# wgurecky/CORRLA_RS

Measured on AMD Instinct MI355X. Metric: RSVD GFLOP/s on 16k x 16k f32 rank-128, higher is better.
Workload: dtype f32

## Files before the change

### corrla_rs_amd/_lib.py

```python
import ctypes as C
import os

PKG = os.path.dirname(os.path.abspath(__file__))
LIB_PATH = os.environ.get("CORRLA_RSVD_LIB") or os.path.join(PKG, "lib", "libcorrla_rsvd.so")

i64, u64, u32, i32, dbl, flt = C.c_int64, C.c_uint64, C.c_uint32, C.c_int32, C.c_double, C.c_float
vp = C.c_void_p

OK, EINVAL, ENOMEM, EHIP, ECOMM, ENUMERIC, ENODEV = range(7)
OMEGA_ON_DEVICE = 0x1
PCA_CENTER_FUSED = 0x2
PCA_CENTER_COPY = 0x4
QR_HOUSEHOLDER = 0x8
SEED_EXPLICIT = 0x10
POWER_FUSED = 0x20
SHARD_COLS = 0x40
SKETCH_BF16X3 = 0x80
SKETCH_BF16X6 = 0x100
PCA_STANDARDIZE = 0x200
COV_CORRELATION = 0x1
COV_NO_CENTER = 0x2
COV_ROUTE_INPLACE, COV_ROUTE_INPLACE_CHECKED, COV_ROUTE_REPACKED = 1, 2, 3
COV_ROUTES = {COV_ROUTE_INPLACE: "inplace", COV_ROUTE_INPLACE_CHECKED: "inplace_checked", COV_ROUTE_REPACKED: "repacked"}
PCA_APPLY_OWN_MEANS = 0x400
# ... 27 lines not shown
                ("scales_out", vp)]


class Timings(C.Structure):
    _fields_ = [("total_ms", dbl), ("sketch_ms", dbl), ("power_ms", dbl), ("qr_ms", dbl), ("project_ms", dbl),
                ("small_svd_ms", dbl), ("finalize_ms", dbl), ("qr_passes", i32), ("n_collectives", i32),
                ("sketch_kernel_ms", dbl), ("host_enqueue_ms", dbl), ("collective_bytes", dbl), ("n_mixed_products", i32),
                ("n_bf16_products", i32), ("knn_ms", dbl), ("fit_ms", dbl)]


def _sigs():
    s = {
        "corrla_version": (C.c_char_p, []),
        "corrla_last_error": (C.c_char_p, []),
        "corrla_device_count": (C.c_int, []),
        "corrla_ctx_create": (C.c_int, [C.c_int, C.POINTER(vp)]),
        "corrla_ctx_destroy": (None, [vp]),
        "corrla_ctx_synchronize": (C.c_int, [vp]),
        "corrla_ctx_get_timings": (C.c_int, [vp, C.POINTER(Timings)]),
        "corrla_ctx_set_phase_timings": (C.c_int, [vp, C.c_int]),
        "corrla_ctx_comm_info": (C.c_int, [vp, C.POINTER(C.c_int), C.POINTER(C.c_int)]),
        "corrla_comm_unique_id": (C.c_int, [vp]),
        "corrla_ctx_comm_init": (C.c_int, [vp, vp, C.c_int, C.c_int]),
        "corrla_ctx_last_pca_apply": (C.c_int, [vp, C.POINTER(C.c_int), C.POINTER(C.c_int)]),
        "corrla_ctx_last_polyfit": (C.c_int, [vp, C.POINTER(C.c_int)]),
        "corrla_ctx_last_kde": (C.c_int, [vp, C.POINTER(C.c_int)]),
        "corrla_ctx_last_dirichlet": (C.c_int, [vp, C.POINTER(C.c_int)]),
        "corrla_ctx_last_mvn": (C.c_int, [vp, C.POINTER(C.c_int)]),
    }
    s["corrla_dirichlet_draws_f64"] = s["corrla_dirichlet_draws_dev_f64"] = (C.c_int, [vp, vp, i64, dbl, u64, i64, i64, vp, i64])
    s["corrla_dirichlet_sample_f64"] = s["corrla_dirichlet_sample_dev_f64"] = (
        C.c_int, [vp, vp, vp, i64, dbl, u64, i64, i64, i64, vp, i64, C.POINTER(i64), C.POINTER(i64)])
    s["corrla_lu_solve_f64"] = (C.c_int, [vp, vp, i64, i64, vp, i64, i64, vp, i64])
    s["corrla_lu_solve_dev_f64"] = (C.c_int, [vp, vp, i64, i64, vp, i64, i64, vp])
    s["corrla_rbffit_system_f64"] = s["corrla_rbffit_system_dev_f64"] = (C.c_int, [vp, vp, i64, i64, i64, C.c_int, dbl, C.c_int, vp, i64])
    s["corrla_rbffit_f64"] = s["corrla_rbffit_dev_f64"] = (C.c_int, [vp, vp, i64, i64, i64, vp, i64, i64, C.c_int, dbl, C.c_int, vp, i64])
    s["corrla_ctx_last_solve"] = (C.c_int, [vp, C.POINTER(C.c_int), C.POINTER(i64), C.POINTER(dbl), C.POINTER(dbl)])
    s["corrla_chol_factor_f64"] = (C.c_int, [vp, vp, i64, i64, vp, i64])
    s["corrla_chol_factor_dev_f64"] = (C.c_int, [vp, vp, i64, i64])
    s["corrla_chol_solve_f64"] = (C.c_int, [vp, vp, i64, i64, vp, i64, i64, vp, i64])
    s["corrla_chol_solve_dev_f64"] = (C.c_int, [vp, vp, i64, i64, vp, i64, i64])
    s["corrla_ctx_last_chol"] = (C.c_int, [vp, C.POINTER(C.c_int), C.POINTER(i64), C.POINTER(dbl), C.POINTER(dbl), C.POINTER(dbl)])
    for suf, sc in (("f32", flt), ("f64", dbl)):
        rsvd = [vp, vp, i64, i64, i64, i64, i64, i64, i64, C.POINTER(Opts), vp, i64, vp, vp, i64]
        s["corrla_rsvd_" + suf] = (C.c_int, rsvd)
        s["corrla_rsvd_dev_" + suf] = (C.c_int, rsvd)
        s["corrla_rsvd_sharded_dev_" + suf] = (C.c_int, rsvd)
        pca = [vp, vp, i64, i64, i64, i64, i64, i64, i64, C.POINTER(Opts), vp, vp, vp, i64]
        s["corrla_pca_" + suf] = (C.c_int, pca)
        s["corrla_pca_dev_" + suf] = (C.c_int, pca)
        s["corrla_pca_sharded_dev_" + suf] = (C.c_int, pca)
        pw = [vp, vp, i64, i64, i64, i64, i64, i64, C.POINTER(Opts), vp, i64]
        s["corrla_power_iter_" + suf] = (C.c_int, pw)
        s["corrla_power_iter_dev_" + suf] = (C.c_int, pw)
        s["corrla_matmul_dev_" + suf] = (C.c_int, [vp, C.c_int, vp, i64, i64, i64, i64, vp, i64, i64, sc, vp, i64])
        rsvd_csr = [vp, vp, vp, vp, i64, i64, i64, i64, i64, i64, C.POINTER(Opts), vp, i64, vp, vp, i64]
        s["corrla_rsvd_csr_" + suf] = (C.c_int, rsvd_csr)
        s["corrla_rsvd_csr_dev_" + suf] = (C.c_int, rsvd_csr)
        pca_csr = [vp, vp, vp, vp, i64, i64, i64, i64, i64, i64, C.POINTER(Opts), vp, vp, vp, i64]
        s["corrla_pca_csr_" + suf] = (C.c_int, pca_csr)
        s["corrla_pca_csr_dev_" + suf] = (C.c_int, pca_csr)
        s["corrla_spmm_csr_dev_" + suf] = (C.c_int, [vp, C.c_int, vp, vp, vp, i64, i64, i64, vp, i64, i64, sc, vp, i64])
        cov = [vp, vp, i64, i64, i64, i64, u64, C.c_int, vp, vp, vp, i64, C.POINTER(C.c_int)]
        s["corrla_cov_" + suf] = (C.c_int, cov)
        s["corrla_cov_dev_" + suf] = (C.c_int, cov)
        model = [vp, vp, vp, i64, i64, u64, vp, i64, vp, vp]
        s["corrla_pca_transform_" + suf] = s["corrla_pca_transform_dev_" + suf] = (C.c_int, [vp, vp, i64, i64, i64, i64] + model)
        s["corrla_pca_transform_csr_" + suf] = s["corrla_pca_transform_csr_dev_" + suf] = (C.c_int, [vp, vp, vp, vp, i64, i64, i64] + model)
        inverse = [vp, vp, i64, i64, i64, vp, vp, vp, i64, i64, vp, i64]
        s["corrla_pca_inverse_" + suf] = s["corrla_pca_inverse_dev_" + suf] = (C.c_int, inverse)
        points = [vp, vp, i64, i64, vp, i64, i64, i64, C.c_int, dbl]
        s["corrla_rbf_matrix_" + suf] = s["corrla_rbf_matrix_dev_" + suf] = (C.c_int, points + [vp, i64])
        s["corrla_rbf_apply_" + suf] = s["corrla_rbf_apply_dev_" + suf] = (C.c_int, points + [C.c_int, vp, i64, i64, vp, i64])
        gram = [vp, vp, i64, i64, i64, vp, i64, i64, C.c_int, C.c_int, vp, i64, vp, vp]
        s["corrla_polyfit_gram_" + suf] = s["corrla_polyfit_gram_dev_" + suf] = (C.c_int, gram)
        peval = [vp, vp, i64, i64, i64, vp, i64, i64, C.c_int, vp, i64, vp, i64]
        s["corrla_poly_eval_" + suf] = s["corrla_poly_eval_dev_" + suf] = (C.c_int, peval)
        kde = [vp, vp, i64, i64, vp, i64, i64]
        s["corrla_kde_eval_" + suf] = s["corrla_kde_eval_dev_" + suf] = (C.c_int, kde + [dbl, C.c_int, vp, i64])
        s["corrla_kde_nll_" + suf] = s["corrla_kde_nll_dev_" + suf] = (C.c_int, kde + [vp, i64, vp, vp])
        s["corrla_mvn_sample_" + suf] = s["corrla_mvn_sample_dev_" + suf] = (C.c_int, [vp, i64, i64, i64, vp, i64, vp, u64, i64, C.c_int, vp, i64])
        s["corrla_sandwich_diag_" + suf] = s["corrla_sandwich_diag_dev_" + suf] = (C.c_int, [vp, vp, i64, i64, i64, vp, i64, vp])
        s["corrla_fill_normal_dev_" + suf] =(C.c_int, [vp, vp, i64, i64, i64, i64, u64, i64, i64])
        s["corrla_time_sketch_dev_" + suf] = (C.c_int, [vp, vp, i64, i64, i64, i64, vp, i64, i64, vp, i64, C.c_int,
                                                         C.POINTER(dbl)])
    s["corrla_rsvd_bf16"] = s["corrla_rsvd_dev_bf16"] = s["corrla_rsvd_f32"]
    s["corrla_pca_bf16"] = s["corrla_pca_dev_bf16"] = s["corrla_pca_f32"]
    s["corrla_matmul_dev_bf16"] = s["corrla_matmul_dev_f32"]
    grad = [vp, vp, i64, i64, vp, vp, i64, C.c_int, i64, dbl, vp, i64, C.POINTER(C.c_int)]
    s["corrla_grad_mat_f64"] = (C.c_int, grad)
    s["corrla_grad_mat_dev_f64"] = (C.c_int, grad)
    return s


SIGNATURES = _sigs()
_lib = None


class CorrlaError(RuntimeError):
    def __init__(self, code, msg):
        super().__init__(f"corrla_rsvd error {code}: {msg}")
        self.code = code


def load():
    global _lib
    if _lib is not None:
        return _lib
    if not os.path.exists(LIB_PATH):
        raise ImportError(
            f"{LIB_PATH} is missing: build it with `python -m corrla_rs_amd.build` (hipcc, gfx950). "
            "corrla_rs_amd has no CPU fallback.")
    try:
        import torch
    except ImportError:
        pass
    lib = C.CDLL(LIB_PATH, mode=C.RTLD_GLOBAL)
    for name, (res, args) in SIGNATURES.items():
        fn = getattr(lib, name)
        fn.restype = res
        fn.argtypes = args
    _lib = lib
    return lib


def check(code):
    if code != OK:
        msg = load().corrla_last_error().decode("utf-8", "replace")
        if code == EINVAL:
            raise ValueError(f"corrla_rsvd: {msg}")
        if code == ENOMEM:
            raise MemoryError(f"corrla_rsvd: {msg}")
        raise CorrlaError(code, msg)
```

### corrla_rs_amd/api.py

```python
import atexit
import ctypes as C
import sys
import threading
import weakref

import numpy as np

from . import _lib as L

__all__ = ["Context", "default_context", "rsvd", "random_svd", "power_iter", "rpca", "PcaRsvd", "algorithmic_flops"]


def _is_torch(x):
    return type(x).__module__.split(".")[0] == "torch"


def _is_torch_csr(x):
    return _is_torch(x) and str(getattr(x, "layout", "")) == "torch.sparse_csr"


def _is_sparse(x):
    if isinstance(x, tuple):
        def nd(v):
            return v.ndim if hasattr(v, "ndim") else np.ndim(v)
# ... 1000 lines not shown
        L.check(self._entry(name, True, in_dtype or xt.dtype)(self._h, 1 if trans else 0, *_c_args(operand), xc.data_ptr(), xin, l, float(beta),
                                                  res.data_ptr(), xout))
        return res.t()

    def spmm(self, a_csr, x, trans=False, beta=1.0):
        import torch
        vals, ci, rp, (m, n), on_dev = _as_csr(a_csr)
        dev = torch.device(f"cuda:{self.device}")
        if not on_dev:
            vals, ci, rp = (torch.from_numpy(v).to(dev) for v in (vals, ci, rp))
        xt = x if _is_torch(x) else torch.as_tensor(np.asarray(x))
        xt = xt.to(device=dev, dtype=vals.dtype)
        if xt.dim() != 2 or xt.shape[0] != (m if trans else n):
            raise ValueError(f"x must have {m if trans else n} rows")
        return self._run_product("corrla_spmm_csr_", (vals, ci, rp, m, n, int(vals.shape[0])),
                                 m, n, xt, trans, beta)

    def matmul(self, a, x, trans=False, beta=1.0):
        m, n = a.shape
        if _is_bf16(x):
            raise ValueError("matmul: x must be float32 or float64 (only the matrix a may be bfloat16)")
        if _is_bf16(a):
            if not str(x.dtype).endswith("float32"):
                raise ValueError("matmul: a bfloat16 a takes a float32 x")
            assert x.shape[0] == (m if trans else n)
            return self._run_product("corrla_matmul_", (a, m, n, *a.stride()), m, n, x, trans, beta, in_dtype=a.dtype)
        assert x.shape[0] == (m if trans else n) and x.dtype == a.dtype
        return self._run_product("corrla_matmul_", (a, m, n, *a.stride()), m, n, x, trans, beta)

    def grad_mat(self, x_mat, y, est_order, n_nbrs, x_query=None, *, scale=1.0):
        est_order, n_nbrs = int(est_order), int(n_nbrs)
        nreg = C.c_int(0)
        if _is_torch(x_mat) and x_mat.is_cuda:
            import torch
            x = x_mat.to(torch.float64).contiguous()
            yv = (y if _is_torch(y) else torch.as_tensor(np.asarray(y))).to(device=x.device, dtype=torch.float64).reshape(-1).contiguous()
            xq = x if x_query is None else x_query.to(device=x.device, dtype=torch.float64).contiguous()
            if x.dim() != 2 or xq.dim() != 2 or xq.shape[1] != x.shape[1] or yv.numel() != x.shape[0]:
                raise ValueError("x_mat (n, k), y (n,), x_query (n_q, k) expected")
            g = torch.empty((xq.shape[0], x.shape[1]), dtype=torch.float64, device=x.device)
            _sync_stream(x)
            L.check(self._lib.corrla_grad_mat_dev_f64(self._h, x.data_ptr(), x.shape[0], x.shape[1], yv.data_ptr(), xq.data_ptr(),
                                                      xq.shape[0], est_order, n_nbrs, float(scale), g.data_ptr(), x.shape[1],
                                                      C.byref(nreg)))
            return g.t(), nreg.value
        x = np.ascontiguousarray(np.asarray(x_mat, dtype=np.float64))
        yv = np.ascontiguousarray(np.asarray(y, dtype=np.float64).reshape(-1))
        xq = x if x_query is None else np.ascontiguousarray(np.asarray(x_query, dtype=np.float64))
        if x.ndim != 2 or xq.ndim != 2 or xq.shape[1] != x.shape[1] or yv.size != x.shape[0]:
            raise ValueError("x_mat (n, k), y (n,), x_query (n_q, k) expected")
        g = np.empty((xq.shape[0], x.shape[1]), dtype=np.float64)
        L.check(self._lib.corrla_grad_mat_f64(self._h, x.ctypes.data, x.shape[0], x.shape[1], yv.ctypes.data, xq.ctypes.data,
                                              xq.shape[0], est_order, n_nbrs, float(scale), g.ctypes.data, x.shape[1],
                                              C.byref(nreg)))
        return g.T, nreg.value

    def power_iter(self, a_mat, omega_rank, n_iter, *, seed=None, omega=None, qr=None):
        _reject_bf16(a_mat, "power_iter")
        a = np.asarray(a_mat)
        if a.ndim != 2:
            raise ValueError("a_mat must be 2-D")
        if a.dtype != np.float32:
            a = a.astype(np.float64, copy=False)
        m, n = a.shape
        w = int(omega_rank)
        rs, cs = _strides(a)
        o, keep = self._opts(seed, omega, n, w, a.dtype, False, self._qr_flag(qr))
        q = _empty_colmajor(a, m, max(w, 1))
        fn = self._entry("corrla_power_iter_", False, a.dtype)
        L.check(fn(self._h, a.ctypes.data, m, n, rs, cs, w, int(n_iter), C.byref(o) if o is not None else None,
                   q.ctypes.data, m))
        del keep
        return q

    def fill_normal(self, t, seed, row0=0, global_cols=None):
        rows, cols = t.shape
        rs, cs = t.stride()
        _sync_stream(t)
        fn = self._entry("corrla_fill_normal_", True, t.dtype)
        L.check(fn(self._h, t.data_ptr(), rows, cols, rs, cs, int(seed), int(row0),
                   int(global_cols if global_cols is not None else cols)))
        return t

    def time_sketch(self, a, x, reps=10):
        import torch
        m, n = a.shape
        rs, cs = a.stride()
        l = x.shape[1]
        xc = x.t().contiguous()
        y = torch.empty((l, m), dtype=a.dtype, device=a.device)
        ms = C.c_double()
        _sync_stream(a)
        fn = self._entry("corrla_time_sketch_", True, a.dtype)
        L.check(fn(self._h, a.data_ptr(), m, n, rs, cs, xc.data_ptr(), n, l, y.data_ptr(), m, int(reps), C.byref(ms)))
        return ms.value, y.t()


_default = None
_default_lock = threading.Lock()


def default_context():
    global _default
    with _default_lock:
        if _default is None:
            _default = Context(0)
        return _default


def rsvd(a_mat, n_rank, n_iters, n_oversamples, *, seed=None, omega=None, ctx=None, qr=None):
    return (ctx or default_context()).rsvd(a_mat, n_rank, n_iters, n_oversamples, seed=seed, omega=omega, qr=qr)


def random_svd(a_mat, omega_rank, n_iter, n_oversamples, *, seed=None, omega=None, ctx=None, qr=None):
    return rsvd(a_mat, omega_rank, n_iter, n_oversamples, seed=seed, omega=omega, ctx=ctx, qr=qr)


def power_iter(a_mat, omega_rank, n_iter, *, seed=None, omega=None, ctx=None, qr=None):
    return (ctx or default_context()).power_iter(a_mat, omega_rank, n_iter, seed=seed, omega=omega, qr=qr)


def rpca(a_mat, n_rank, n_iters=None, n_oversamples=None, *, seed=None, omega=None, ctx=None, standardize=False):
    del n_iters, n_oversamples
    if not _check_standardize(standardize):
        _means, s, comps = (ctx or default_context()).pca(a_mat, n_rank, seed=seed, omega=omega)
    else:
        _means, s, comps, _scales = (ctx or default_context()).pca(a_mat, n_rank, seed=seed, omega=omega, standardize=True)
    return s, comps


def normal_stream_host(seed, first, n, r, dtype=np.float64):
    dtype = np.dtype(dtype)
    if dtype not in (np.float32, np.float64):
        raise ValueError(f"dtype must be float32 or float64, got {dtype}")
    n, r, seed, first = int(n), int(r), int(seed), int(first)
    if n < 0 or r < 1 or first < 0 or (first + n) * r >= 1 << 63:
        raise ValueError("need n >= 0, r >= 1, first >= 0 and (first + n) * r < 2^63")
    m32, sh = np.uint64(0xFFFFFFFF), np.uint64(32)
    t = (np.uint64(first) + np.arange(n, dtype=np.uint64))[:, None] * np.uint64(r) + np.arange(r, dtype=np.uint64)[None, :]
    c0, c1, c2, c3 = t & m32, t >> sh, np.zeros_like(t), np.zeros_like(t)
    k0, k1 = np.uint64(seed & 0xFFFFFFFF), np.uint64((seed >> 32) & 0xFFFFFFFF)
    for _ in range(10):
        p0, p1 = np.uint64(0xD2511F53) * c0, np.uint64(0xCD9E8D57) * c2
        c0, c1, c2, c3 = (p1 >> sh) ^ c1 ^ k0, p1 & m32, (p0 >> sh) ^ c3 ^ k1, p0 & m32
        k0, k1 = (k0 + np.uint64(0x9E3779B9)) & m32, (k1 + np.uint64(0xBB67AE85)) & m32
    if dtype == np.float64:
        u1 = ((((c0 << sh) | c1) >> np.uint64(11)).astype(np.float64) + 0.5) * 2.0 ** -53
        u2 = ((((c2 << sh) | c3) >> np.uint64(11)).astype(np.float64) + 0.5) * 2.0 ** -53
    else:
        u1 = ((c0 >> np.uint64(8)).astype(np.float32) + np.float32(0.5)) * np.float32(2.0 ** -24)
        u2 = ((c1 >> np.uint64(8)).astype(np.float32) + np.float32(0.5)) * np.float32(2.0 ** -24)
    x = dtype.type(2.0) * u2
    y = np.where(x > 1.0, dtype.type(2.0) - x, x)
    pi = dtype.type(np.pi)
    c = np.where(y < 0.25, np.cos(pi * y), np.where(y > 0.75, -np.cos(pi * (dtype.type(1.0) - y)), np.sin(pi * (dtype.type(0.5) - y))))
    return (np.sqrt(dtype.type(-2.0) * np.log(u1)) * c).astype(dtype)


class PcaRsvd:

    def __init__(self, x_mat, rank, *, seed=None, omega=None, ctx=None, standardize=False):
        self.pca_rank = int(rank)
        x = x_mat if _is_sparse(x_mat) or (_is_torch(x_mat) and x_mat.is_cuda) else np.asarray(x_mat)
        self._ctx = ctx
        self.n_samples = int(x[3][0] if isinstance(x, tuple) else x.shape[0])
        self.scales_ = None
# ... 83 lines not shown
```

### corrla_rs_amd/csrc/capi_impl.hpp

```cpp
#pragma once
#include <cstddef>
#include <cstdint>
#include <cstring>
#include <string>
#include <vector>

#include "../../include/corrla_rsvd.h"
#include "call_spans.hpp"
#include "driver.hpp"
#include "rbf_plan.hpp"
#include "polyfit_plan.hpp"
#include "kde_plan.hpp"
#include "dirichlet_plan.hpp"
#include "mvn_plan.hpp"
#include "chol_plan.hpp"
#include "lu_plan.hpp"

namespace corrla {

inline std::string& last_error_slot() {
  static thread_local std::string msg;
  return msg;
}

// ... 140 lines not shown
    dev.begin_call();
    begun = true;
    stage();
  };
  if (!sharded) {
    prepare();
    return;
  }
  if (dev.nranks() < 1) throw Error(ST_ECOMM, "communicator not initialised");
  int local = ST_OK;
  std::string local_msg;
  try {
    prepare();
  } catch (const Error& e) {
    local = e.code;
    local_msg = e.what();
  } catch (const std::bad_alloc&) {
    local = ST_ENOMEM;
    local_msg = "host allocation failed";
  }
  if (!begun) dev.begin_call();
  const int agreed = dev.sharded_handshake(local);
  if (local != ST_OK) throw Error(local, local_msg);
  if (agreed != ST_OK)
    throw Error(agreed, "sharded call abandoned: another rank failed before the first collective (status " + std::to_string(agreed) +
                            "); this rank's arguments were valid");
}

template <class Dev, class T>
inline void finish_call(RsvdDriver<Dev, T>& drv, Dev& dev, Timings* tm_out, bool with_sketch_kernel_ms) {
  PhaseTimer fin;
  drv.phase(drv.tm.finalize_ms, fin);
  dev.phase_end();
  dev.end_call();
  dev.phase_resolve(&drv.tm.total_ms);
  drv.tm.n_collectives = dev.n_collectives;
  drv.tm.collective_bytes = dev.collective_bytes;
  if (with_sketch_kernel_ms) drv.tm.sketch_kernel_ms = dev.event_elapsed_ms(0, 1);
  if (tm_out) *tm_out = drv.tm;
}

template <class T>
struct RsvdCall {
  bool host_ptrs;
  int64_t m, rank, n_iter, n_oversamples;
  const corrla_opts* opts;
  T* u;
  int64_t ldu;
  T* s;
  T* vt;
  int64_t ldvt;
  Timings* tm_out;
  bool profile;
  bool sharded = false, sparse = false, fat = false, empty_shard = false;
  bool bf16 = false;
};

template <class Dev, class T, class Validate, class Stage>
inline void rsvd_body(Dev& dev, const RsvdCall<T>& c, Validate&& validate, Stage&& stage) {
  const bool shard_cols = c.sharded && c.fat;
  const int64_t k = c.rank;
  RunOpts ro;
  TallA<T> ta;
  bool u_in_place = false;
  int64_t l = 0;
  Skinny<T> ut, vtall;
  T* s_dev = nullptr;
  prepare_call(
      dev, c.sharded,
      [&] {
        if ((!c.u && !(c.empty_shard && !shard_cols)) || !c.s || (!c.vt && !(c.empty_shard && shard_cols)))
          throw Error(ST_EINVAL, "output pointer is NULL");
        validate();
        if (c.ldu < c.m) throw Error(ST_EINVAL, "ldu < m");
        if (c.ldvt < c.rank) throw Error(ST_EINVAL, "ldvt < rank");
        ro = call_opts(c.opts, c.host_ptrs, c.sharded, c.sparse || c.bf16);
        draw_seed(dev, ro);
      },
      [&] {
        ta = stage();
        l = std::min<int64_t>(c.rank + c.n_oversamples, ta.nt);
        if (ro.omega && ro.omega_ld < ta.nt) throw Error(ST_EINVAL, "omega_ld < min(m, n)");
        u_in_place = !c.fat && !c.host_ptrs && !c.empty_shard;
        ut = u_in_place ? caller_skinny(c.u, ta.mt, k, c.ldu) : dev.template alloc_skinny<T>(ta.mt, k);
        vtall = dev.template alloc_skinny<T>(ta.nt, k);
        s_dev = dev.template alloc_scalar<T>((int)k);
      });
  RsvdDriver<Dev, T> drv(dev, c.profile);
  if (c.empty_shard) drv.m_local_override_ = 0;
  drv.random_svd_tall(ta, k, l, c.n_iter, ro, ut, s_dev, vtall, [&] {
    if (!c.fat) {
      if (!u_in_place && !c.empty_shard) dev.copy_out(ut, k, c.u, c.ldu, false, c.host_ptrs);
      dev.copy_out(vtall, k, c.vt, c.ldvt, true, c.host_ptrs);
    } else {
      dev.copy_out(vtall, k, c.u, c.ldu, false, c.host_ptrs);
      if (!c.empty_shard) dev.copy_out(ut, k, c.vt, c.ldvt, true, c.host_ptrs);
    }
    dev.copy_values_out(s_dev, k, c.s, c.host_ptrs);
  });
  finish_call(drv, dev, c.tm_out, true);
}

template <class Dev, class T>
inline void rsvd_entry(Dev& dev, bool host_ptrs, bool sharded, const T* a, int64_t m, int64_t n, int64_t rs, int64_t cs,
                       int64_t rank, int64_t n_iter, int64_t n_oversamples, const corrla_opts* opts, T* u, int64_t ldu,
                       T* s, T* vt, int64_t ldvt, Timings* tm_out, bool profile) {
  const bool shard_cols = sharded && opts && (opts->flags & CORRLA_SHARD_COLS) != 0;
  const bool empty_shard = sharded && m >= 0 && n >= 0 && (shard_cols ? (n == 0 && m >= 1) : (m == 0 && n >= 1));
  const int64_t short_side = shard_cols ? m : n;
  RsvdCall<T> c{host_ptrs, m, rank, n_iter, n_oversamples, opts, u, ldu, s, vt, ldvt, tm_out, profile};
  c.sharded = sharded;
  c.fat = sharded ? shard_cols : m < n;
  c.empty_shard = empty_shard;
  rsvd_body(
      dev, c,
      [&] {
        if (!empty_shard) validate_matrix(a, m, n, rs, cs);
        if (!sharded && opts && (opts->flags & CORRLA_SHARD_COLS)) throw Error(ST_EINVAL, "CORRLA_SHARD_COLS is only valid for sharded entry points");
        if (sharded) {
          if (rank < 1 || rank > short_side) throw Error(ST_EINVAL, "rank must be in [1, short side] for the sharded path");
          if (n_iter < 0 || n_oversamples < 0) throw Error(ST_EINVAL, "n_iter and n_oversamples must be >= 0");
        } else {
          validate_rank(m, n, rank, n_iter, n_oversamples);
        }
      },
      [&] {
        if (empty_shard) return zero_row_tall<Dev, T>(dev, short_side);
        return shard_cols ? stage_input<Dev, T>(dev, host_ptrs, a, n, m, cs, rs, true)
                          : stage_input<Dev, T>(dev, host_ptrs, a, m, n, rs, cs, sharded);
      });
}

inline void need_two_samples(int64_t m) {
  if (m < 2) throw Error(ST_EINVAL, "PCA needs at least two samples");
}

template <class T>
struct PcaCall {
  bool host_ptrs;
  int64_t m, n, rank, n_iter, n_oversamples;
  const corrla_opts* opts;
  T* means;
  T* s;
  T* comps;
  int64_t ldc;
  Timings* tm_out;
  bool profile;
  bool sharded = false, sparse = false;
  bool bf16 = false;
};

template <class Dev, class T, class Validate, class Stage>
inline void pca_body(Dev& dev, const PcaCall<T>& c, Validate&& validate, Stage&& stage) {
  RunOpts ro;
  TallA<T> ta;
  T* scales_out = nullptr;
  prepare_call(
      dev, c.sharded,
      [&] {
        if (!c.means || !c.s || !c.comps) throw Error(ST_EINVAL, "output pointer is NULL");
        validate();
        if (c.ldc < c.rank) throw Error(ST_EINVAL, "ldc < rank");
        if (c.sparse) need_two_samples(c.m);
        ro = call_opts(c.opts, c.host_ptrs, c.sharded, c.sparse || c.bf16, true);
        if (ro.pca_standardize && !dev_has_colvar<Dev>::value)
          throw Error(ST_EINVAL, "CORRLA_PCA_STANDARDIZE: this backend has no column-variance kernels");
        if (ro.pca_standardize && c.opts->struct_size >= sizeof(corrla_opts)) scales_out = (T*)c.opts->scales_out;
        if (c.sparse && ro.pca_center == 2)
          throw Error(ST_EINVAL, "CORRLA_PCA_CENTER_COPY on CSR input: a centred copy would densify the matrix (use the fused centring)");
        draw_seed(dev, ro);
      },
      [&] { ta = stage(); });
  const int64_t m_global = c.sharded ? dev.allreduce_sum_host(c.m) : c.m;
  need_two_samples(m_global);
  const bool fat = !c.sharded && c.m < c.n;
  RsvdDriver<Dev, T> drv(dev, c.profile);
  Skinny<T> mu = drv.column_means(ta, fat, m_global, c.sharded);
  const bool data_cols_along_mem_cols = (ta.row_major != fat);
  Skinny<T> sd, inv_sd;
  if (ro.pca_standardize) {
    if constexpr (dev_has_colvar<Dev>::value) {
// ... 939 lines not shown
```

### corrla_rs_amd/csrc/core_svd_stage.hpp

```cpp
#pragma once
#include "core_svd_plan.hpp"
#include "hip_backend.hpp"

namespace corrla {

template <class T>
struct CoreSvdCall {
  const Skinny<T>& c;
  int64_t l, k;
  Skinny<T>&m1, &m2;
  T* s_dev;
  void* conv_status;
};

namespace core_svd_stage {

template <class T>
using RingEs = std::integer_sequence<int, 8, 12, 16, sizeof(T) == 4 ? 20 : 18>;
constexpr int kMaxNc = 9;

template <class T>
inline void set_lds_limits() {
  for_each_of(RingEs<T>{}, [](auto e) { lds_limit((const void*)k::jacobi_ring_w_kernel<T, decltype(e)::value, 8>, k::kLdsMaxBytes); });
  lds_limit((const void*)k::jacobi_block_round_kernel<T>, k::kLdsMaxBytes);
// ... 78 lines not shown
  int* bad = a.conv_status ? nullptr : dev.alloc_flags(1);
  hipLaunchKernelGGL((k::core_finite_check_kernel<T>), dim3(1), dim3(1024), 0, dev.stream, (const T*)a.c.p, a.c.ld, (int)a.l,
                     (k::CholStatus*)a.conv_status, bad, sexp_out);
  CORRLA_HIP(hipGetLastError());
  if (bad) {
    int h = 0;
    dev.read_flags(bad, 1, &h);
    if (h) throw Error(ST_ENUMERIC, "non-finite core matrix in small SVD");
  }
}

template <class T>
inline void block(HipDev& dev, const CoreSvdCall<T>& a, const CoreSvdPlan& plan, const int* sexp) {
  const CoreSvdPlan::Block& p = plan.blk;
  const int64_t ld = p.rows_pad;
  T* wj = (T*)dev.alloc_bytes(p.ws_bytes);
  T* vj = (T*)dev.alloc_bytes(p.ws_bytes);
  k::JacobiCtl* ctl = (k::JacobiCtl*)dev.alloc_bytes(sizeof(k::JacobiCtl));
  hipLaunchKernelGGL((k::jacobi_init_kernel<T>), dim3(64), dim3(256), 0, dev.stream, (const T*)a.c.p, a.c.ld, (int)a.l, wj, ld, vj,
                     ld, p.cols_pad, p.rows_pad, ctl, sexp);
  for (int sw = 0; sw < p.max_sweeps; ++sw) {
    for (int round = 0; round < p.nb - 1; ++round)
      hipLaunchKernelGGL((k::jacobi_block_round_kernel<T>), dim3(p.nb / 2), dim3(256), p.round_lds, dev.stream, wj, ld, vj, ld,
                         p.rows_pad, p.nb, round, p.inner, ctl);
    hipLaunchKernelGGL(k::jacobi_sweep_end_kernel, dim3(1), dim3(1), 0, dev.stream, ctl, (float)plan.tol_early);
  }
  hipLaunchKernelGGL((k::jacobi_finish_kernel<T>), dim3(1), dim3(1024), p.fin_lds, dev.stream, (const T*)wj, ld, (const T*)vj,
                     ld, (int)a.l, a.m1.p, a.m1.ld, a.m2.p, a.m2.ld, a.s_dev, (int)a.k, sexp);
  CORRLA_HIP(hipGetLastError());
  if (env_int("CORRLA_DEBUG", 0)) {
    k::JacobiCtl h;
    CORRLA_HIP(hipMemcpyAsync(&h, ctl, sizeof(h), hipMemcpyDeviceToHost, dev.stream));
    dev.sync();
    std::fprintf(stderr, "[corrla] block jacobi l=%d nb=%d sweeps=%u done=%u\n", (int)a.l, p.nb, h.sweeps, h.done);
  }
}

template <class T>
inline void ring(HipDev& dev, const CoreSvdCall<T>& a, const CoreSvdPlan& plan) {
  static_assert(sizeof(k::RotEntry<T>) == 2 * sizeof(T), "CoreSvdPlan::Ring::rot_bytes");
  const CoreSvdPlan::Ring& p = plan.ring;
  int* info = (int*)dev.alloc_bytes(sizeof(int) * 4);
  k::RotEntry<T>* rot = (k::RotEntry<T>*)dev.alloc_bytes(p.rot_bytes);
  int* rank_g = (int*)dev.alloc_bytes(p.rank_bytes);
  const T tol = (T)plan.tol, tol_early = (T)plan.tol_early;
  with_one_of(RingEs<T>{}, plan.ring_e, [&](auto e) {
    hipLaunchKernelGGL((k::jacobi_ring_w_kernel<T, decltype(e)::value, 8>), dim3(1), dim3(p.block), p.lds, dev.stream, (const T*)a.c.p,
                       a.c.ld, (int)a.l, a.m2.p, a.m2.ld, a.s_dev, (int)a.k, tol, tol_early, p.max_sw, rot, rank_g, info);
  });
  CORRLA_HIP(hipGetLastError());
  hipLaunchKernelGGL((k::jacobi_replay_v_kernel<T>), dim3(p.replay_grid), dim3(256), 0, dev.stream, (const k::RotEntry<T>*)rot,
                     (const int*)info, (const int*)rank_g, (int)a.l, (int)a.k, a.m1.p, a.m1.ld);
  CORRLA_HIP(hipGetLastError());
  if (env_int("CORRLA_DEBUG", 0)) {
    int h[4] = {0, 0, 0, 0};
    CORRLA_HIP(hipMemcpyAsync(h, info, sizeof(int), hipMemcpyDeviceToHost, dev.stream));
    dev.sync();
    std::fprintf(stderr, "[corrla] jacobi_svd (ring) l=%d sweeps=%d\n", (int)a.l, h[0]);
  }
}

inline CoreSvdKnobs knobs_from_env() {
  CoreSvdKnobs kn;
  kn.mode = std::getenv("CORRLA_SVD");
  kn.host_svd = env_int("CORRLA_HOST_SVD", 0) != 0;
  kn.jmc_min_l = env_int("CORRLA_JMC_MIN_L", kn.jmc_min_l);
  kn.jmc_max_b = std::min(32, std::max(2, env_int("CORRLA_JMC_MAX_B", kn.jmc_max_b)));
  kn.jmc_local = env_int("CORRLA_JMC_LOCAL", kn.jmc_local);
  kn.jmc_np = env_int("CORRLA_JMC_NP", kn.jmc_np);
  kn.jmc_sweeps_f32 = env_int("CORRLA_JMC_SWEEPS", kn.jmc_sweeps_f32);
  kn.jmc_sweeps_f64 = env_int("CORRLA_JMC_SWEEPS", kn.jmc_sweeps_f64);
  kn.jmc_force_v = env_int("CORRLA_JMC_FORCE_V", 0) != 0;
  kn.strict = env_int("CORRLA_JACOBI_STRICT", 0) != 0;
  kn.block_sweeps = env_int("CORRLA_JACOBI_SWEEPS", kn.block_sweeps);
  kn.ring_sweeps = env_int("CORRLA_JACOBI_SWEEPS", kn.ring_sweeps);
  kn.block_inner = env_int("CORRLA_JACOBI_INNER", kn.block_inner);
  return kn;
}

}

template <class T>
void HipDev::small_svd(const Skinny<T>& c, int64_t l, int64_t k, Skinny<T>& m1, Skinny<T>& m2, T* s_dev, void* conv_status) {
  if (conv_status) memset_zero(conv_status, sizeof(k::CholStatus));
  const CoreSvdCall<T> a{c, l, k, m1, m2, s_dev, conv_status};
  const CoreSvdPlan plan = core_svd_plan((int)sizeof(T), l, k, core_svd_stage::knobs_from_env(), svd_state_, conv_status != nullptr);
  switch (plan.family) {
    case CoreSvd::kMultiWg:
      core_svd_stage::multi_wg(*this, a, plan);
      return;
    case CoreSvd::kHost:
      small_svd_host(*this, c, l, k, m1, m2, s_dev);
      return;
    case CoreSvd::kBlock: {
      int* sexp = (int*)alloc_bytes(sizeof(int));
      core_svd_stage::finite_check(*this, a, sexp);
      core_svd_stage::block(*this, a, plan, sexp);
      return;
    }
    case CoreSvd::kRing:
      core_svd_stage::finite_check(*this, a);
      core_svd_stage::ring(*this, a, plan);
      return;
  }
}

}
```

### corrla_rs_amd/csrc/corrla_rsvd.hip

```cpp
#include <mutex>

#include "capi_impl.hpp"
#include "colstat_stage.hpp"
#include "core_svd_stage.hpp"
#include "cov_stage.hpp"
#include "dirichlet_stage.hpp"
#include "grad_stage.hpp"
#include "hip_backend.hpp"
#include "kde_stage.hpp"
#include "chol_stage.hpp"
#include "lu_stage.hpp"
#include "mvn_stage.hpp"
#include "pca_apply_stage.hpp"
#include "polyfit_stage.hpp"
#include "rbf_stage.hpp"
#include "tall_stage.hpp"
#include "thinq_stage.hpp"

using namespace corrla;

struct corrla_ctx {
  HipDev dev;
  Timings last;
  std::mutex mu;
  bool profile;
  pca_apply_stage::Ran pca_apply;
  polyfit_stage::Ran polyfit;
  kde_stage::Ran kde;
  dirichlet_stage::Ran dirichlet;
  mvn_stage::Ran mvn;
  lu_stage::Ran lu;
  chol_stage::Ran chol;
  explicit corrla_ctx(int ordinal) : dev(ordinal), profile(env_int("CORRLA_PROFILE_PHASES", 0) != 0) {}
};

namespace {
inline corrla_ctx* need(corrla_ctx* c) {
  if (!c) throw Error(ST_EINVAL, "ctx is NULL");
  return c;
}
template <class F>
inline void locked_call(corrla_ctx* c, F&& f) {
  std::lock_guard<std::mutex> lk(c->mu);
  try {
    f();
  } catch (...) {
    (void)hipSetDevice(c->dev.device);
    if (c->dev.stream) (void)hipStreamSynchronize(c->dev.stream);
    (void)hipGetLastError();
    throw;
  }
}

template <class F, class After>
inline corrla_status ctx_call(corrla_ctx* ctx, F&& f, After&& after) {
  return guarded([&] {
    corrla_ctx* c = need(ctx);
    locked_call(c, [&] { f(*c); });
    after(*c);
  });
}
template <class F>
inline corrla_status ctx_call(corrla_ctx* ctx, F&& f) {
  return ctx_call(ctx, f, [](corrla_ctx&) {});
}
inline void debug_qr_breakdown(const corrla_ctx& c) {
  if (c.profile && env_int("CORRLA_DEBUG", 0))
    std::fprintf(stderr, "[corrla] qr breakdown (ms): gram %.3f  download+check %.3f  host chol/inv %.3f  upload+apply %.3f  (%d passes)\n",
                 c.last.qr_gram_ms, c.last.qr_down_ms, c.last.qr_host_ms, c.last.qr_apply_ms, c.last.qr_passes);
}
template <class T>
corrla_status fill_c(corrla_ctx* ctx, T* p, int64_t rows, int64_t cols, int64_t rs, int64_t cs, uint64_t seed,
                     int64_t row0, int64_t global_cols) {
  return guarded([&] {
    corrla_ctx* c = need(ctx);
    if (!p) throw Error(ST_EINVAL, "p is NULL");
    if (rows < 0 || cols < 0 || rs < 0 || cs < 0 || global_cols < cols) throw Error(ST_EINVAL, "bad fill_normal shape");
    std::lock_guard<std::mutex> lk(c->mu);
    CORRLA_HIP(hipSetDevice(c->dev.device));
    c->dev.fill_normal(p, rows, cols, rs, cs, seed, row0, global_cols);
    c->dev.sync();
  });
}
template <class T>
corrla_status time_sketch_c(corrla_ctx* ctx, const T* a, int64_t m, int64_t n, int64_t rs, int64_t cs, const T* x,
                            int64_t ldx, int64_t l, T* y, int64_t ldy, int reps, double* avg_ms) {
  return guarded([&] {
    corrla_ctx* c = need(ctx);
    if (!x || !y || !avg_ms) throw Error(ST_EINVAL, "NULL argument");
    if (reps < 1 || l < 1 || ldx < n || ldy < m) throw Error(ST_EINVAL, "bad time_sketch arguments");
    std::lock_guard<std::mutex> lk(c->mu);
    HipDev& dev = c->dev;
    dev.begin_call();
    TallA<T> ta = stage_input<HipDev, T>(dev, false, a, m, n, rs, cs, true);
    RsvdDriver<HipDev, T> drv(dev, false);
    drv.mixed_planes_ = parse_opts(nullptr, true).mixed_planes;
    Skinny<T> xs = dev.alloc_skinny<T>(n, l);
    dev.copy_in_skinny(x, ldx, xs);
    Skinny<T> out = dev.alloc_skinny<T>(m, l);
    *avg_ms = dev.time_on_stream(reps, [&] { drv.a_times(ta, xs, out, nullptr); });
    dev.copy_out(out, l, y, ldy, false, false);
    dev.end_call();
  });
}
}

extern "C" {

CORRLA_API const char* corrla_version(void) { return "corrla_rsvd 0.1.0 gfx950"; }
CORRLA_API const char* corrla_last_error(void) { return last_error_slot().c_str(); }
CORRLA_API int corrla_device_count(void) {
  int n = 0;
  if (hipGetDeviceCount(&n) != hipSuccess) {
    (void)hipGetLastError();
    return 0;
  }
  return n;
}

CORRLA_API corrla_status corrla_ctx_create(int device_ordinal, corrla_ctx** out) {
  return guarded([&] {
    if (!out) throw Error(ST_EINVAL, "out is NULL");
    *out = nullptr;
    *out = new corrla_ctx(device_ordinal);
  });
}
CORRLA_API void corrla_ctx_destroy(corrla_ctx* ctx) { delete ctx; }
CORRLA_API corrla_status corrla_ctx_synchronize(corrla_ctx* ctx) {
  return guarded([&] { need(ctx)->dev.sync(); });
}
CORRLA_API corrla_status corrla_ctx_comm_info(corrla_ctx* ctx, int* rank, int* nranks) {
  return guarded([&] {
    corrla_ctx* c = need(ctx);
    if (!rank || !nranks) throw Error(ST_EINVAL, "NULL argument");
    std::lock_guard<std::mutex> lk(c->mu);
    c->dev.comm_info(rank, nranks);
  });
}
CORRLA_API corrla_status corrla_ctx_set_phase_timings(corrla_ctx* ctx, int on) {
  return guarded([&] {
    corrla_ctx* c = need(ctx);
    std::lock_guard<std::mutex> lk(c->mu);
    c->dev.set_phase_events(on != 0);
  });
}
CORRLA_API corrla_status corrla_ctx_get_timings(corrla_ctx* ctx, corrla_timings* out) {
  return guarded([&] {
    corrla_ctx* c = need(ctx);
    if (!out) throw Error(ST_EINVAL, "out is NULL");
    const Timings& t = c->last;
    out->total_ms = t.total_ms;
    out->sketch_ms = t.sketch_ms;
    out->power_ms = t.power_ms;
    out->qr_ms = t.qr_ms;
    out->project_ms = t.project_ms;
    out->small_svd_ms = t.small_svd_ms;
    out->finalize_ms = t.finalize_ms;
    out->qr_passes = t.qr_passes;
    out->n_collectives = t.n_collectives;
    out->collective_bytes = t.collective_bytes;
    out->sketch_kernel_ms = t.sketch_kernel_ms;
    out->host_enqueue_ms = t.host_enqueue_ms;
    out->n_mixed_products = t.n_mixed_products;
    out->n_bf16_products = t.n_bf16_products;
    out->knn_ms = t.knn_ms;
    out->fit_ms = t.fit_ms;
  });
}

#define CORRLA_DENSE(T, A) const T *A, int64_t m, int64_t n, int64_t rs, int64_t cs
#define CORRLA_CSR_A(T) const T *values, const int32_t *col_idx, const int64_t *row_ptr, int64_t m, int64_t n, int64_t nnz
#define CORRLA_RSVD_REST(T) int64_t rank, int64_t n_iter, int64_t p, const corrla_opts *o, T *u, int64_t ldu, T *s, T *vt, int64_t ldvt
#define CORRLA_PCA_REST(T) int64_t rank, int64_t n_iter, int64_t p, const corrla_opts *o, T *means, T *s, T *comps, int64_t ldc
#define CORRLA_PRODUCT_REST(T) const T *x, int64_t ldx, int64_t l, T beta, T *res, int64_t ldres

#define CORRLA_DEFINE_RSVD(NAME, T, HOST, SHARDED)                                                                      \
  CORRLA_API corrla_status NAME(corrla_ctx* ctx, CORRLA_DENSE(T, a), CORRLA_RSVD_REST(T)) {                              \
    return ctx_call(ctx, [&](corrla_ctx& c) {                                                                           \
      rsvd_entry<HipDev, T>(c.dev, HOST, SHARDED, a, m, n, rs, cs, rank, n_iter, p, o, u, ldu, s, vt, ldvt, &c.last,     \
                            c.profile);                                                                                 \
    }, debug_qr_breakdown);                                                                                             \
  }
#define CORRLA_DEFINE_PCA(NAME, T, HOST, SHARDED)                                                                       \
  CORRLA_API corrla_status NAME(corrla_ctx* ctx, CORRLA_DENSE(T, x), CORRLA_PCA_REST(T)) {                             \
    return ctx_call(ctx, [&](corrla_ctx& c) {                                                                           \
      pca_entry<HipDev, T>(c.dev, HOST, x, m, n, rs, cs, rank, n_iter, p, o, means, s, comps, ldc, &c.last, c.profile,   \
                           SHARDED);                                                                                    \
    });                                                                                                                 \
  }
#define CORRLA_DEFINE_POWER(NAME, T, HOST)                                                                              \
  CORRLA_API corrla_status NAME(corrla_ctx* ctx, CORRLA_DENSE(T, a), int64_t width, int64_t n_iter, const corrla_opts* o, \
                                T* q, int64_t ldq) {                                                                    \
    return ctx_call(ctx, [&](corrla_ctx& c) {                                                                           \
      power_iter_entry<HipDev, T>(c.dev, HOST, a, m, n, rs, cs, width, n_iter, o, q, ldq);                              \
    });                                                                                                                 \
  }

#define CORRLA_DEFINE(SUF, T)                                                                                          \
  CORRLA_DEFINE_RSVD(corrla_rsvd_##SUF, T, true, false)                                                                \
  CORRLA_DEFINE_RSVD(corrla_rsvd_dev_##SUF, T, false, false)                                                           \
  CORRLA_DEFINE_RSVD(corrla_rsvd_sharded_dev_##SUF, T, false, true)                                                    \
  CORRLA_DEFINE_PCA(corrla_pca_##SUF, T, true, false)                                                                  \
  CORRLA_DEFINE_PCA(corrla_pca_dev_##SUF, T, false, false)                                                             \
  CORRLA_DEFINE_PCA(corrla_pca_sharded_dev_##SUF, T, false, true)                                                      \
  CORRLA_DEFINE_POWER(corrla_power_iter_##SUF, T, true)                                                                \
  CORRLA_DEFINE_POWER(corrla_power_iter_dev_##SUF, T, false)                                                           \
  CORRLA_API corrla_status corrla_matmul_dev_##SUF(corrla_ctx* ctx, int trans, CORRLA_DENSE(T, a), CORRLA_PRODUCT_REST(T)) { \
    return ctx_call(ctx, [&](corrla_ctx& c) {                                                                          \
      matmul_entry<HipDev, T>(c.dev, trans, a, m, n, rs, cs, x, ldx, l, beta, res, ldres, &c.last);                    \
    });                                                                                                                \
  }                                                                                                                    \
  CORRLA_API corrla_status corrla_fill_normal_dev_##SUF(corrla_ctx* ctx, T* p, int64_t rows, int64_t cols, int64_t rs,            \
                                             int64_t cs, uint64_t seed, int64_t row0, int64_t global_cols) {           \
    return fill_c<T>(ctx, p, rows, cols, rs, cs, seed, row0, global_cols);                                             \
  }                                                                                                                    \
  CORRLA_API corrla_status corrla_time_sketch_dev_##SUF(corrla_ctx* ctx, const T* a, int64_t m, int64_t n, int64_t rs,            \
                                             int64_t cs, const T* x, int64_t ldx, int64_t l, T* y, int64_t ldy,        \
                                             int reps, double* avg_ms) {                                               \
    return time_sketch_c<T>(ctx, a, m, n, rs, cs, x, ldx, l, y, ldy, reps, avg_ms);                                    \
  }

CORRLA_DEFINE(f32, float)
CORRLA_DEFINE(f64, double)

#define CORRLA_DEFINE_RSVD_CSR(NAME, T, HOST)                                                                           \
  CORRLA_API corrla_status NAME(corrla_ctx* ctx, CORRLA_CSR_A(T), CORRLA_RSVD_REST(T)) {                                \
    return ctx_call(ctx, [&](corrla_ctx& c) {                                                                           \
      rsvd_csr_entry<HipDev, T>(c.dev, HOST, values, col_idx, row_ptr, m, n, nnz, rank, n_iter, p, o, u, ldu, s, vt,     \
                                ldvt, &c.last, c.profile);                                                              \
    });                                                                                                                 \
  }
#define CORRLA_DEFINE_PCA_CSR(NAME, T, HOST)                                                                            \
  CORRLA_API corrla_status NAME(corrla_ctx* ctx, CORRLA_CSR_A(T), CORRLA_PCA_REST(T)) {                                 \
    return ctx_call(ctx, [&](corrla_ctx& c) {                                                                           \
      pca_csr_entry<HipDev, T>(c.dev, HOST, values, col_idx, row_ptr, m, n, nnz, rank, n_iter, p, o, means, s, comps,    \
                               ldc, &c.last, c.profile);                                                                \
    });                                                                                                                 \
  }

#define CORRLA_DEFINE_CSR(SUF, T)                                                                                      \
  CORRLA_DEFINE_RSVD_CSR(corrla_rsvd_csr_##SUF, T, true)                                                               \
  CORRLA_DEFINE_RSVD_CSR(corrla_rsvd_csr_dev_##SUF, T, false)                                                          \
  CORRLA_DEFINE_PCA_CSR(corrla_pca_csr_##SUF, T, true)                                                                 \
  CORRLA_DEFINE_PCA_CSR(corrla_pca_csr_dev_##SUF, T, false)                                                            \
  CORRLA_API corrla_status corrla_spmm_csr_dev_##SUF(corrla_ctx* ctx, int trans, CORRLA_CSR_A(T), CORRLA_PRODUCT_REST(T)) { \
    return ctx_call(ctx, [&](corrla_ctx& c) {                                                                          \
      spmm_entry<HipDev, T>(c.dev, trans, values, col_idx, row_ptr, m, n, nnz, x, ldx, l, beta, res, ldres);           \
    });                                                                                                                \
  }

CORRLA_DEFINE_CSR(f32, float)
CORRLA_DEFINE_CSR(f64, double)

#define CORRLA_DEFINE_RSVD_BF16(NAME, HOST)                                                                             \
  CORRLA_API corrla_status NAME(corrla_ctx* ctx, CORRLA_DENSE(uint16_t, a), CORRLA_RSVD_REST(float)) {                  \
    return ctx_call(ctx, [&](corrla_ctx& c) {                                                                           \
      rsvd_bf16_entry<HipDev>(c.dev, HOST, a, m, n, rs, cs, rank, n_iter, p, o, u, ldu, s, vt, ldvt, &c.last, c.profile); \
    });                                                                                                                 \
  }
#define CORRLA_DEFINE_PCA_BF16(NAME, HOST)                                                                              \
  CORRLA_API corrla_status NAME(corrla_ctx* ctx, CORRLA_DENSE(uint16_t, x), CORRLA_PCA_REST(float)) {                   \
    return ctx_call(ctx, [&](corrla_ctx& c) {                                                                           \
      pca_bf16_entry<HipDev>(c.dev, HOST, x, m, n, rs, cs, rank, n_iter, p, o, means, s, comps, ldc, &c.last, c.profile); \
    });                                                                                                                 \
  }
CORRLA_DEFINE_RSVD_BF16(corrla_rsvd_bf16, true)
CORRLA_DEFINE_RSVD_BF16(corrla_rsvd_dev_bf16, false)
CORRLA_DEFINE_PCA_BF16(corrla_pca_bf16, true)
CORRLA_DEFINE_PCA_BF16(corrla_pca_dev_bf16, false)
CORRLA_API corrla_status corrla_matmul_dev_bf16(corrla_ctx* ctx, int trans, CORRLA_DENSE(uint16_t, a), CORRLA_PRODUCT_REST(float)) {
  return ctx_call(ctx, [&](corrla_ctx& c) {
    matmul_bf16_entry<HipDev>(c.dev, trans, a, m, n, rs, cs, x, ldx, l, beta, res, ldres, &c.last);
  });
}

#define CORRLA_DEFINE_COV(NAME, T, HOST)                                                                                \
  CORRLA_API corrla_status NAME(corrla_ctx* ctx, CORRLA_DENSE(T, x), uint64_t flags, int ddof, T* means_out, T* scales_out, \
                                T* c, int64_t ldc, int* route_out) {                                                    \
    return ctx_call(ctx, [&](corrla_ctx& cx) {                                                                          \
      const CovCall<T> call{x, m, n, rs, cs, flags, ddof, means_out, scales_out, c, ldc, route_out};                    \
      cov_entry<HipDev, T>(cx.dev, call, [&] { cov_stage::run<T>(cx.dev, HOST, call); });                               \
    });                                                                                                                 \
  }
CORRLA_DEFINE_COV(corrla_cov_f32, float, true)
CORRLA_DEFINE_COV(corrla_cov_f64, double, true)
CORRLA_DEFINE_COV(corrla_cov_dev_f32, float, false)
CORRLA_DEFINE_COV(corrla_cov_dev_f64, double, false)

#define CORRLA_PCA_MODEL(T) const T *means, const T *scales, const T *components, int64_t ldc, int64_t k, uint64_t flags, T *scores, \
                            int64_t ld_scores, T *resid_out, T *means_out
#define CORRLA_PCA_MODEL_CALL(T) PcaTransformCall<T>{m, n, means, scales, components, ldc, k, flags, scores, ld_scores, resid_out, means_out}
#define CORRLA_DEFINE_PCA_TRANSFORM(NAME, T, HOST)                                                                      \
  CORRLA_API corrla_status NAME(corrla_ctx* ctx, CORRLA_DENSE(T, x), CORRLA_PCA_MODEL(T)) {                             \
    return ctx_call(ctx, [&](corrla_ctx& cx) {                                                                          \
      cx.pca_apply = pca_apply_stage::Ran();                                                                            \
      const PcaTransformCall<T> c = CORRLA_PCA_MODEL_CALL(T);                                                           \
      if (!x) throw Error(ST_EINVAL, "pca_transform: x is NULL");                                                       \
      if (m < 1 || n < 1) throw Error(ST_EINVAL, "pca_transform: m and n must be >= 1");                                \
// ... 323 lines not shown
```

### corrla_rs_amd/csrc/driver.hpp

```cpp
#pragma once
#include <cstdio>
#include <chrono>
#include <cmath>
#include <cstdint>
#include <cstring>
#include <limits>
#include <stdexcept>
#include <string>
#include <functional>
#include <type_traits>
#include <vector>

#include "gemm_plan.hpp"
#include "small_linalg.hpp"
#include "thinq_plan.hpp"

namespace corrla {

struct Error : std::runtime_error {
  int code;
  Error(int c, const std::string& m) : std::runtime_error(m), code(c) {}
};
enum { ST_OK = 0, ST_EINVAL = 1, ST_ENOMEM = 2, ST_EHIP = 3, ST_ECOMM = 4, ST_ENUMERIC = 5, ST_ENODEV = 6 };

// ... 15 lines not shown
template <class T>
struct Big {
  const T* p = nullptr;
  int64_t rows = 0, cols = 0, ld = 0, cols_readable = 0;
};

template <class T>
inline Big<T> as_rowmajor_transposed(const Skinny<T>& y, int64_t ncols) {
  Big<T> b;
  b.p = y.p;
  b.rows = ncols;
  b.cols = y.rows;
  b.ld = y.ld;
  b.cols_readable = y.ld;
  return b;
}

template <class T>
struct CsrView {
  const T* val = nullptr;
  const int32_t* ci = nullptr;
  const int64_t* rp = nullptr;
  int64_t rows = 0, cols = 0, nnz = 0;
  int64_t n_long = 0, n_chunks = 0;
  const int64_t* long_row = nullptr;
  const int64_t* long_base = nullptr;
  const int32_t* chunk_long = nullptr;
};

template <class D, class = void>
struct dev_has_spmm : std::false_type {};
template <class D>
struct dev_has_spmm<D, std::void_t<decltype(D::kHasSpmm)>> : std::true_type {};

template <class D, class = void>
struct dev_has_bf16in : std::false_type {};
template <class D>
struct dev_has_bf16in<D, std::void_t<decltype(D::kHasBf16In)>> : std::true_type {};

template <class D, class = void>
struct dev_has_colvar : std::false_type {};
template <class D>
struct dev_has_colvar<D, std::void_t<decltype(D::kHasColVar)>> : std::true_type {};

template <class D, class = void>
struct dev_has_syrk : std::false_type {};
template <class D>
struct dev_has_syrk<D, std::void_t<decltype(D::kHasSyrk)>> : std::true_type {};

template <class D, class = void>
struct dev_has_pca_apply : std::false_type {};
template <class D>
struct dev_has_pca_apply<D, std::void_t<decltype(D::kHasPcaApply)>> : std::true_type {};

template <class D, class = void>
struct dev_has_rbf : std::false_type {};
template <class D>
struct dev_has_rbf<D, std::void_t<decltype(D::kHasRbf)>> : std::true_type {};

template <class D, class = void>
struct dev_has_polyfit : std::false_type {};
template <class D>
struct dev_has_polyfit<D, std::void_t<decltype(D::kHasPolyfit)>> : std::true_type {};
template <class D, class = void>
struct dev_has_kde : std::false_type {};
template <class D>
struct dev_has_kde<D, std::void_t<decltype(D::kHasKde)>> : std::true_type {};
template <class D, class = void>
struct dev_has_dirichlet : std::false_type {};
template <class D>
struct dev_has_dirichlet<D, std::void_t<decltype(D::kHasDirichlet)>> : std::true_type {};
template <class D, class = void>
struct dev_has_mvn : std::false_type {};
template <class D>
struct dev_has_mvn<D, std::void_t<decltype(D::kHasMvn)>> : std::true_type {};
template <class D, class = void>
struct dev_has_lu : std::false_type {};
template <class D>
struct dev_has_lu<D, std::void_t<decltype(D::kHasLu)>> : std::true_type {};
template <class D, class = void>
struct dev_has_chol : std::false_type {};
template <class D>
struct dev_has_chol<D, std::void_t<decltype(D::kHasChol)>> : std::true_type {};

template <class T>
struct TallA {
  Big<T> mem;
  bool row_major = true;
  int64_t mt = 0, nt = 0;
  const T* mu_short = nullptr;
  const T* mu_tall = nullptr;
  const T* inv_sd_short = nullptr;
  const T* inv_sd_tall = nullptr;
  bool sparse = false;
  CsrView<T> csr, csr_t;
  bool bf16 = false;
  Big<uint16_t> mem16;
};

struct RunOpts {
  uint64_t seed = 0x5eedull;
  bool seed_explicit = false;
  const void* omega = nullptr;
  int64_t omega_ld = 0;
  bool omega_on_device = false;
  bool sharded = false;
  int pca_center = 0;
  bool pca_standardize = false;
  bool qr_householder = false;
  bool power_fused = false;
  int mixed_planes = 0;
  bool mixed_project = true;
  int poison_core = 0;
};
constexpr int kFlagNonFinite = 2, kFlagNullCols = 4;

struct Timings {
  double total_ms = 0, sketch_ms = 0, power_ms = 0, qr_ms = 0, project_ms = 0, small_svd_ms = 0, finalize_ms = 0;
  double host_enqueue_ms = 0;
  int qr_passes = 0;
  int n_collectives = 0;
  double collective_bytes = 0;
  double knn_ms = 0, fit_ms = 0;
  int n_mixed_products = 0;
  int n_bf16_products = 0;
  double qr_gram_ms = 0, qr_down_ms = 0, qr_host_ms = 0, qr_apply_ms = 0;
  double sketch_kernel_ms = 0;
};

struct PhaseTimer {
  using clk = std::chrono::steady_clock;
  clk::time_point t0;
  PhaseTimer() : t0(clk::now()) {}
  double lap() {
    auto t1 = clk::now();
    double ms = std::chrono::duration<double, std::milli>(t1 - t0).count();
    t0 = t1;
    return ms;
  }
};

template <class Dev, class T>
struct RsvdDriver {
  Dev& dev;
  Timings tm;
  bool profile_phases;
  bool qr_householder = false;
  static constexpr const T* kNone = nullptr;

  explicit RsvdDriver(Dev& d, bool profile = false) : dev(d), profile_phases(profile) {}

  int mixed_planes_ = 0;
  void sparse_times(const CsrView<T>& s, const Skinny<T>& x, Skinny<T>& y, const T* scale_dev) {
    if constexpr (dev_has_spmm<Dev>::value)
      dev.spmm(s, x, y, scale_dev);
    else
      throw Error(ST_EINVAL, "this backend has no SpMM kernels: sparse operands are not supported");
  }
  void bf16_times(bool tn, const Big<uint16_t>& r, const Skinny<T>& x, Skinny<T>& y, const T* scale_dev) {
    if constexpr (dev_has_bf16in<Dev>::value && std::is_same<T, float>::value)
      dev.gemm_bf16a(tn, r, x, y, scale_dev), ++tm.n_bf16_products;
    else
      throw Error(ST_EINVAL, "this backend has no bf16-input kernels: bf16 operands are not supported");
  }
  Skinny<T> scale_ws_;
  void set_scale_workspace(const Skinny<T>& ws) { scale_ws_ = ws; }
// ... 96 lines not shown
      p.record = record;
      return p;
    }
  };
  struct Attempt {
    bool defer = false;
    void* st_pool = nullptr;
    int st_slots = 0, st_used = 0;
    int* flags_pool = nullptr;
    int flags_cap = 0, flags_used = 0;
    std::vector<Pending> pending;
    bool dirty = false;
  } att_;
  void* status_record(int i) const { return (char*)att_.st_pool + (size_t)i * kStatusBytes; }
  int64_t m_local_ = 0, m_global_ = -1;
  int64_t m_local_override_ = -1;
  int64_t global_rows(bool sharded) {
    if (!sharded) return m_local_;
    if (m_global_ < 0) m_global_ = dev.allreduce_sum_host(m_local_);
    return m_global_;
  }

  int hh_short_shards_ = -1;
  bool householder_usable(const Skinny<T>& y, bool sharded) {
    if (!qr_householder) return false;
    if (!sharded) return y.rows >= y.cols;
    if (hh_short_shards_ < 0) hh_short_shards_ = (int)dev.allreduce_sum_host(m_local_ < y.cols ? 1 : 0);
    return hh_short_shards_ == 0;
  }
  void householder_panel(Skinny<T>& y, Skinny<T>& tmp, bool sharded) {
    const int64_t l = y.cols;
    auto h = dev.householder_up(y, tmp);
    if (!sharded) {
      dev.householder_down(h, y, tmp);
      return;
    }
    const int64_t np = dev.nranks(), rk = dev.rank();
    Skinny<T> stack = dev.template alloc_skinny<T>(np * l, l), t2 = dev.template alloc_skinny<T>(np * l, l);
    Skinny<T> rv, cv;
    rv.p = h.r_root();
    rv.rows = rv.cols = rv.ld = rv.cols_alloc = l;
    dev.copy_block(rv, 0, 0, l, l, stack, rk * l, 0);
    dev.allreduce(stack.p, (size_t)stack.ld * (size_t)stack.cols_alloc);
    dev.householder_thin_q(stack, t2);
    cv.p = (T*)dev.alloc_zeroed_bytes((size_t)l * (size_t)l * sizeof(T));
    cv.rows = cv.cols = cv.ld = cv.cols_alloc = l;
    dev.copy_block(stack, rk * l, 0, l, l, cv, 0, 0);
    dev.householder_down(h, y, tmp, (const T*)cv.p);
  }
  void householder_thin_q_any_width(Skinny<T>& y, Skinny<T>& tmp, bool sharded) {
    const int64_t l = y.cols, m = y.rows;
    const int64_t w = hh_column_blocks(l, dev.template householder_max_width<T>()).w;
    if (w == l) {
      householder_panel(y, tmp, sharded);
      return;
    }
    std::vector<double> th;
    for (int64_t c0 = 0; c0 < l; c0 += w) {
      const int64_t wb = std::min(w, l - c0);
      Skinny<T> yb = dev.template alloc_skinny<T>(m, wb), tb = dev.template alloc_skinny<T>(m, wb);
      Skinny<T> pb = dev.template alloc_skinny<T>(m, wb);
      dev.copy_block(y, 0, c0, m, wb, yb, 0, 0);
      for (int pass = 0; pass < 5; ++pass) {
        double overlap2 = 0.0;
        if (c0 > 0) {
          Skinny<T> t = dev.template alloc_skinny<T>(c0, wb);
          dev.gemm_nn(as_rowmajor_transposed(y, c0), yb, t, kNone);
          if (sharded) dev.allreduce(t.p, (size_t)t.ld * (size_t)t.cols_alloc);
          if (pass >= 1) {
            th.resize((size_t)(c0 * wb));
            dev.download_skinny(t, c0, wb, th.data());
            for (double v : th) overlap2 += v * v;
          }
          dev.gemm_tn(as_rowmajor_transposed(y, c0), t, pb, kNone);
          dev.sub_inplace(yb, pb);
        }
        householder_panel(yb, tb, sharded);
        if (c0 == 0 || (pass >= 1 && overlap2 <= 0.25)) break;
      }
      dev.copy_block(yb, 0, 0, m, wb, y, 0, c0);
    }
  }

  int64_t orthonormalize(Skinny<T>& y, Skinny<T>& tmp, bool sharded, bool rough = false) {
    const int64_t l = y.cols;
    if (householder_usable(y, sharded)) {
      PhaseTimer qt0;
      householder_thin_q_any_width(y, tmp, sharded);
      ++tm.qr_passes;
      subphase(tm.qr_gram_ms, qt0);
      return l;
    }
    int64_t r = orthonormalize_core(y, tmp, sharded, rough);
    if (r < l && !att_.defer && (sharded ? global_rows(true) : y.rows) >= l) r = complete_basis(y, r, sharded);
    return r;
  }

  int64_t complete_basis(Skinny<T>& y, int64_t r, bool sharded) {
    const int64_t l = y.cols, c = l - r, m = y.rows;
    Skinny<T> yc = dev.template alloc_skinny<T>(m, c);
    Skinny<T> pc = dev.template alloc_skinny<T>(m, c);
    Skinny<T> tc = dev.template alloc_skinny<T>(m, c);
    dev.fill_normal(yc.p, m, c, (int64_t)1, yc.ld, (uint64_t)(0x9e3779b97f4a7c15ull ^ (uint64_t)(131 * r + l)), (int64_t)0, c);
    if (r > 0) {
      for (int pass = 0; pass < 2; ++pass) {
        Skinny<T> t = dev.template alloc_skinny<T>(r, c);
        dev.gemm_nn(as_rowmajor_transposed(y, r), yc, t, kNone);
        if (sharded) dev.allreduce(t.p, (size_t)t.ld * (size_t)t.cols_alloc);
        dev.gemm_tn(as_rowmajor_transposed(y, r), t, pc, kNone);
        dev.sub_inplace(yc, pc);
      }
    }
    const int64_t rc = orthonormalize_core(yc, tc, sharded, false);
    dev.copy_cols(yc, y, r, rc);
    return r + rc;
  }

  template <class Factor>
  void cholqr_pass(Skinny<T>& y, Skinny<T>& tmp, Skinny<T>& gd, bool sharded, bool inplace, Factor&& factor) {
    const int64_t l = y.cols;
    Skinny<T> yv = y.view_cols(l);
    dev.gemm_nn(as_rowmajor_transposed(y, l), yv, gd, kNone);
    if (sharded) dev.allreduce(gd.p, (size_t)gd.ld * (size_t)gd.cols_alloc);
    const Skinny<T> md = factor(gd);
    if (inplace) {
      dev.apply_inplace(y, l, md);
    } else {
      dev.gemm_tn(as_rowmajor_transposed(y, l), md, tmp, kNone);
      std::swap(y.p, tmp.p);
    }
  }

  struct BlockSplit {
    int64_t n1 = 0, n2 = 0;
    T* minus_one = nullptr;
  };
  int records_per_pass(int64_t l) const {
    return dev.template device_chol_fits<T>(l) ? 1 : (dev.template device_chol_blocked_fits<T>(l) ? 2 : 0);
  }
  BlockSplit block_split(int64_t l) {
    BlockSplit s;
    s.n1 = blocked_split_n1(l);
    s.n2 = l - s.n1;
    s.minus_one = dev.template alloc_scalar<T>(1);
    dev.fill_const(s.minus_one, (int64_t)1, (T)-1);
    return s;
  }
  template <class Factor>
  void blocked_factor_inverse(const Skinny<T>& g, const BlockSplit& s, Skinny<T>& md, Factor&& factor) {
    const int64_t n1 = s.n1, n2 = s.n2;
    Skinny<T> g11 = dev.template alloc_skinny<T>(n1, n1), g12 = dev.template alloc_skinny<T>(n1, n2);
    Skinny<T> g22 = dev.template alloc_skinny<T>(n2, n2), x11 = dev.template alloc_skinny<T>(n1, n1);
    Skinny<T> x22 = dev.template alloc_skinny<T>(n2, n2), r12 = dev.template alloc_skinny<T>(n1, n2);
    Skinny<T> t22 = dev.template alloc_skinny<T>(n2, n2), t12 = dev.template alloc_skinny<T>(n1, n2);
    Skinny<T> x12 = dev.template alloc_skinny<T>(n1, n2);
    dev.copy_block(g, 0, 0, n1, n1, g11, 0, 0);
    dev.copy_block(g, 0, n1, n1, n2, g12, 0, 0);
    dev.copy_block(g, n1, n1, n2, n2, g22, 0, 0);
    factor(g11, n1, 0, x11);
    dev.gemm_nn(as_rowmajor_transposed(x11, n1), g12, r12, kNone);
    dev.gemm_nn(as_rowmajor_transposed(r12, n2), r12, t22, kNone);
    dev.sub_inplace(g22, t22);
    factor(g22, n2, 1, x22);
    dev.gemm_tn(as_rowmajor_transposed(r12, n2), x22, t12, kNone);
    dev.gemm_tn(as_rowmajor_transposed(x11, n1), t12, x12, s.minus_one);
    dev.copy_block(x11, 0, 0, n1, n1, md, 0, 0);
    dev.copy_block(x12, 0, 0, n1, n2, md, 0, n1);
    dev.copy_block(x22, 0, 0, n2, n2, md, n1, n1);
  }

  int64_t orthonormalize_device(Skinny<T>& y, Skinny<T>& tmp, bool sharded, bool rough, bool polish) {
    const int64_t l = y.cols;
    PhaseTimer qt0;
    const bool inplace = dev.qr_inplace_fits(l), single = dev.template device_chol_fits<T>(l);
    const RobustSchedule sched =
        robust_schedule(dev.robust_passes(), polish ? RobustMode::kPolish : (rough ? RobustMode::kInLoop : RobustMode::kFinal), inplace);
    const int npass = sched.npass, always = sched.always;
    int* need = att_.flags_pool + att_.flags_used;
    int* null_mask = dev.alloc_flags((int)l);
    int* need_blk = dev.alloc_flags(2);
    void* st_scratch = dev.alloc_zeroed_bytes((size_t)2 * npass * kStatusBytes);
    void* insp = single ? nullptr : dev.template alloc_inspect<T>();
    Skinny<T> gd = dev.template alloc_skinny<T>(l, l);
    Skinny<T> md = dev.template alloc_skinny<T>(l, l);
    double shift_rel = robust_shift_rel(sizeof(T), y.rows, l, single);
    if (const char* e = std::getenv("CORRLA_QR_SHIFT_SCALE")) shift_rel *= std::atof(e);
    float nullx = 1.f;
    if (const char* e = std::getenv("CORRLA_QR_NULL_EXCESS")) nullx = (float)std::atof(e);
    const BlockSplit split = single ? BlockSplit{} : block_split(l);
    for (int pass = 0; pass < npass; ++pass) {
      const RobustSchedule::Pass& ps = sched.pass[pass];
      dev.set_run_if(ps.gate < 0 ? nullptr : need + ps.gate);
      const float nx = ps.null_excess ? nullx : 0.f;
      cholqr_pass(y, tmp, gd, sharded, inplace, [&](Skinny<T>& g) {
        if (single) {
          dev.chol_inv_robust(g, l, kPivotTol, (float)shift_rel, ps.shift_mode, nx, md, st_scratch, pass, need + pass, null_mask, nullptr,
                              ps.need_ratio);
          return md;
        }
        dev.gram_inspect(g, l, (float)shift_rel, ps.shift_mode, insp);
        const void* shp = dev.template inspect_shift_ptr<T>(insp);
        blocked_factor_inverse(g, split, md, [&](const Skinny<T>& blk, int64_t n, int which, Skinny<T>& x) {
          dev.chol_inv_robust(blk, n, kPivotTol, 0.f, 2, nx, x, st_scratch, 2 * pass + which, need_blk + which,
                              null_mask + which * split.n1, shp, ps.need_ratio);
        });
        dev.template combine_need<T>(need + pass, ps.need_ratio > 0.f ? nullptr : insp, need_blk, need_blk + 1);
        return md;
      });
      if (ps.refill)
        dev.refill_null(y, l, null_mask, (uint64_t)(0x9e3779b97f4a7c15ull ^ (uint64_t)(977 * (att_.flags_used + pass) + l)));
      if (pass < always) ++tm.qr_passes;
    }
    dev.set_run_if(nullptr);
    att_.pending.push_back(Pending::robust_chol(always, npass, sched.flag_slot < 0 ? -1 : att_.flags_used + sched.flag_slot, st_scratch,
                                                single ? 1 : 2));
    att_.flags_used += npass;
    subphase(tm.qr_gram_ms, qt0);
    return l;
  }

  int64_t orthonormalize_core(Skinny<T>& y, Skinny<T>& tmp, bool sharded, bool rough, bool polish = false) {
    const int64_t l = y.cols;
    int64_t r = l;
    if (att_.defer && (sharded || y.rows >= l) && att_.flags_used + kRobustPasses <= att_.flags_cap &&
        dev.template device_qr_robust_fits<T>(l))
      return orthonormalize_device(y, tmp, sharded, rough, polish);
    const int rpp = records_per_pass(l);
    if (rpp > 0) {
      PhaseTimer qt0;
      const int npass = rough ? 1 : 2, nrec = npass * rpp;
      Skinny<T> gd0 = dev.template alloc_skinny<T>(l, l);
      Skinny<T> md0 = rpp == 1 ? dev.template alloc_skinny<T>(l, l) : Skinny<T>{};
      const bool defer = att_.defer && att_.st_used + nrec <= att_.st_slots;
      void* st_dev = defer ? status_record(att_.st_used) : dev.alloc_bytes((size_t)2 * rpp * kStatusBytes);
      const BlockSplit split = rpp == 1 ? BlockSplit{} : block_split(l);
      for (int pass = 0; pass < npass; ++pass) {
        cholqr_pass(y, tmp, gd0, sharded, false, [&](Skinny<T>& g) {
          if (rpp == 1) {
            dev.chol_inv(g, l, kPivotTol, md0, st_dev, pass);
            return md0;
          }
          Skinny<T> md = dev.template alloc_skinny<T>(l, l);
          blocked_factor_inverse(g, split, md, [&](const Skinny<T>& blk, int64_t n, int which, Skinny<T>& x) {
            dev.chol_inv(blk, n, kPivotTol, x, st_dev, 2 * pass + which);
          });
          return md;
        });
        ++tm.qr_passes;
      }
      if (defer) {
        att_.pending.push_back(Pending::optimistic_chol(att_.st_used, npass, rpp, !rough));
        att_.st_used += nrec;
        subphase(tm.qr_gram_ms, qt0);
        return l;
      }
      int fail[4] = {0, 0, 0, 0};
      float min_ratio[4], dev_i[4];
      dev.read_chol_status(st_dev, nrec, fail, min_ratio, dev_i);
      subphase(tm.qr_gram_ms, qt0);
      bool ok = true;
      for (int i = 0; i < nrec; ++i) {
        if (fail[i] == 3) throw Error(ST_ENUMERIC, "non-finite Gram matrix in orthonormalisation");
        ok = ok && fail[i] == 0;
      }
      if (rpp == 1 && fail[0] == 2) return 0;
      for (int i = nrec - rpp; !rough && i < nrec; ++i) ok = ok && dev_i[i] <= 0.25f;
      if (ok) return l;
    }
    if (att_.defer) att_.dirty = true;
    const double eps = (double)std::numeric_limits<T>::epsilon();
    std::vector<double> g((size_t)l * l), mm((size_t)l * l), uu, ss, vv;
    Skinny<T> gd = dev.template alloc_skinny<T>(l, l);
    Skinny<T> md = dev.template alloc_skinny<T>(l, l);
    int fails = 0;
    bool series_next = false;
    const double series_max_e = sizeof(T) == 4 ? 1e-2 : 1e-4;
    for (int pass = 0; pass < 12; ++pass) {
      if (r == 0) break;
      Skinny<T> yv = y.view_cols(r);
      Skinny<T> gv = gd.view_cols(r);
      gv.rows = r;
      PhaseTimer qt;
      dev.gemm_nn(as_rowmajor_transposed(y, r), yv, gv, kNone);
      if (sharded) dev.allreduce(gd.p, (size_t)gd.ld * (size_t)gd.cols_alloc);
      subphase(tm.qr_gram_ms, qt);
      ++tm.qr_passes;
      if (series_next) {
        Skinny<T> mv = md.view_cols(r);
        mv.rows = r;
        dev.inv_sqrt_series(gv, r, mv);
        Skinny<T> out = tmp.view_cols(r);
        dev.gemm_tn(as_rowmajor_transposed(y, r), mv, out, kNone);
        if (r < l) dev.zero_cols(tmp, r, l);
        std::swap(y.p, tmp.p);
        subphase(tm.qr_apply_ms, qt);
        break;
      }
      dev.download_skinny(gv, r, r, g.data());
      double gmax = 0.0, dev_i = 0.0;
      for (int64_t j = 0; j < r; ++j)
        for (int64_t i = 0; i < r; ++i) {
          const double x = g[(size_t)j * r + i];
          if (!std::isfinite(x)) throw Error(ST_ENUMERIC, "non-finite Gram matrix in orthonormalisation");
          dev_i = std::max(dev_i, std::fabs(x - (i == j ? 1.0 : 0.0)));
          if (i == j) gmax = std::max(gmax, x);
        }
      if (gmax == 0.0) {
        r = 0;
        break;
      }
      subphase(tm.qr_down_ms, qt);
      if (dev_i <= 16.0 * eps) break;
      const bool near_i = dev_i <= 0.25;
      int64_t r_new = r;
      bool clean = false;
      double min_ratio_last = 0.0;
      if (fails >= 3) {
        uu.resize((size_t)r * r);
        vv.resize((size_t)r * r);
        ss.resize(r);
        if (small::jacobi_svd((int)r, g.data(), (int)r, uu.data(), ss.data(), vv.data(), 1e-15) < 0)
          throw Error(ST_ENUMERIC, "non-finite Gram matrix in orthonormalisation");
        r_new = 0;
        while (r_new < r && ss[r_new] > 1e-2 * ss[0]) ++r_new;
        std::fill(mm.begin(), mm.end(), 0.0);
        for (int64_t j = 0; j < r_new; ++j) {
          const double sc = 1.0 / std::sqrt(ss[j]);
          for (int64_t i = 0; i < r; ++i) mm[(size_t)j * r + i] = vv[(size_t)j * r + i] * sc;
        }
        fails = 0;
      } else {
        std::vector<double> rr(g.begin(), g.begin() + (size_t)r * r);
        double min_ratio = 0.0;
        clean = small::chol_upper((int)r, rr.data(), (int)r, 4.0 * eps, &min_ratio);
        min_ratio_last = min_ratio;
        if (!clean) {
          ++fails;
          double shift = 16.0 * eps * gmax;
          bool ok = false;
          for (int tries = 0; tries < 8 && !ok; ++tries, shift *= 10.0) {
            rr.assign(g.begin(), g.begin() + (size_t)r * r);
            for (int64_t i = 0; i < r; ++i) rr[(size_t)i * r + i] += shift;
            ok = small::chol_upper((int)r, rr.data(), (int)r, 0.0, &min_ratio);
          }
          if (!ok) throw Error(ST_ENUMERIC, "Gram matrix not positive definite even after shifting");
        } else {
          fails = 0;
        }
        small::triu_inverse((int)r, rr.data(), (int)r);
        std::copy(rr.begin(), rr.end(), mm.begin());
      }
      subphase(tm.qr_host_ms, qt);
      Skinny<T> mv = md.view_cols(r_new);
      mv.rows = r;
      dev.upload_skinny(mm.data(), r, r_new, r, md);
      Skinny<T> out = tmp.view_cols(r_new);
      dev.gemm_tn(as_rowmajor_transposed(y, r), mv, out, kNone);
      if (r_new < l) dev.zero_cols(tmp, r_new, l);
      std::swap(y.p, tmp.p);
      r = r_new;
      subphase(tm.qr_apply_ms, qt);
      if (clean && (near_i || rough)) break;
      if (clean && fails == 0 && r == l && 4.0 * (double)l * eps / std::max(min_ratio_last, 1e-300) <= series_max_e)
        series_next = true;
    }
    return r;
  }

  int64_t power_iter(const TallA<T>& a, int64_t l, int64_t n_iter, const RunOpts& o, Skinny<T>& y, Skinny<T>& y2) {
    qr_householder = o.qr_householder;
    m_local_ = m_local_override_ >= 0 ? m_local_override_ : a.mt;
    struct MixedScope {
      int& slot;
      int saved;
      MixedScope(int& s, int v) : slot(s), saved(s) { slot = v; }
      ~MixedScope() { slot = saved; }
    } mixed_scope(mixed_planes_, o.mixed_planes);
    PhaseTimer pt;
    Skinny<T> om = dev.template alloc_skinny<T>(a.nt, l);
    if (o.omega) {
      if (o.omega_on_device)
        dev.copy_in_skinny((const T*)o.omega, o.omega_ld, om);
      else
        dev.upload_skinny_native((const T*)o.omega, o.omega_ld, om);
    } else {
      dev.fill_normal(om.p, a.nt, l, 1, om.ld, o.seed, 0, l);
    }
    Skinny<T> z = dev.template alloc_skinny<T>(a.nt, l);
    double* ss_dev = dev.alloc_f64(1);
    T* inv_dev = dev.template alloc_scalar<T>(1);
    int64_t i0 = 0;
    const bool fused = o.power_fused && n_iter > 0 && !a.sparse && a.row_major && !a.mu_short && !a.mu_tall &&
                       dev.template ata_fused_fits<T>(a.mem, l);
    if (fused) {
      const int64_t nf = std::min<int64_t>(n_iter, 3);
      for (int64_t i = 0; i < nf; ++i) {
        if (i == 0) dev.event_mark(0);
        dev.ata_fused(a.mem, i == 0 ? om : z, z);
        if (i == 0) dev.event_mark(1);
        if (o.sharded) dev.allreduce(z.p, (size_t)z.ld * (size_t)z.cols);
        dev.inv_norm(z, ss_dev, inv_dev);
        dev.scale_inplace(z, inv_dev);
        if (i == 0) phase(tm.sketch_ms, pt);
      }
      a_times(a, z, y, kNone);
      i0 = nf;
    } else {
      dev.event_mark(0);
      a_times(a, om, y, kNone);
      dev.event_mark(1);
      phase(tm.sketch_ms, pt);
    }
    for (int64_t i = i0; i < n_iter; ++i) {
      if (i > 2) {
        phase(tm.power_ms, pt);
        orthonormalize(y, y2, o.sharded, true);
        phase(tm.qr_ms, pt);
      }
      at_times(a, y, z, kNone, o.sharded);
      dev.inv_norm(z, ss_dev, inv_dev);
      dev.scale_inplace(z, inv_dev);
      a_times(a, z, y, kNone);
    }
    phase(tm.power_ms, pt);
    int64_t r = orthonormalize(y, y2, o.sharded);
    phase(tm.qr_ms, pt);
    return r;
  }

  void random_svd_tall(const TallA<T>& a, int64_t k, int64_t l, int64_t n_iter, const RunOpts& o, Skinny<T>& u_tall,
                       T* s_dev, Skinny<T>& v_tall, const std::function<void()>& emit = {}) {
    qr_householder = o.qr_householder;
    m_local_ = m_local_override_ >= 0 ? m_local_override_ : a.mt;
    m_global_ = -1;
    hh_short_shards_ = -1;
    const bool hh = qr_householder;
    if (!hh && records_per_pass(l) > 0) {
      const Timings saved = tm;
      const auto mark = dev.arena_mark();
      bool on_device = true;
      for (int attempt = 0; attempt < 5 && on_device; ++attempt) {
        if (attempt > 0) dev.arena_rewind(mark);
        att_ = Attempt{};
        att_.st_slots = (int)std::min<int64_t>(4 * (std::max<int64_t>(0, n_iter - 3) + 2) + 1, 4096);
        att_.flags_cap = kRobustPasses * (int)std::min<int64_t>(std::max<int64_t>(0, n_iter - 3) + 4, 1024);
        att_.st_pool = dev.alloc_zeroed_bytes((size_t)att_.st_slots * kStatusBytes + (size_t)att_.flags_cap * sizeof(int));
        att_.flags_pool = (int*)status_record(att_.st_slots);
        att_.defer = true;
        try {
          random_svd_tall_body(a, k, l, n_iter, o, u_tall, s_dev, v_tall);
        } catch (...) {
          att_.defer = false;
          throw;
        }
        att_.defer = false;
        if (emit) emit();
        const Verdict verdict = attempt_verdict();
        if (verdict == Verdict::kClean) return;
        tm = saved;
        dev.phase_forget();
        switch (verdict) {
          case Verdict::kMorePasses:
            on_device = dev.robust_passes() < kRobustPasses;
            if (on_device) dev.set_robust_passes(std::min(kRobustPasses, 2 * std::max(2, dev.robust_passes())));
            break;
          case Verdict::kMoreSweeps:
            on_device = dev.svd_more_sweeps();
            break;
          case Verdict::kNeedV:
            on_device = dev.svd_force_v();
            break;
// ... 3 lines not shown
      }
      dev.arena_rewind(mark);
    }
    random_svd_tall_body(a, k, l, n_iter, o, u_tall, s_dev, v_tall);
    if (emit) emit();
  }

  enum class Verdict { kClean, kRepeatOnHost, kMorePasses, kMoreSweeps, kNeedV };
  struct StatusRecord {
    int fail;
    float min_ratio, dev_i, gmax;
    long long clk, wall;
  };
  static_assert(sizeof(StatusRecord) == kStatusBytes, "status record layout");
  static void debug_record(int i, const char* what, const StatusRecord& r) {
    if (std::getenv("CORRLA_DEBUG"))
      std::fprintf(stderr, "[corrla] status record %d (%s): fail %d min_ratio %.3g dev_i %.3g\n", i, what, r.fail, r.min_ratio, r.dev_i);
  }
  Verdict attempt_verdict() {
    const Attempt& at = att_;
    if (at.dirty) return Verdict::kRepeatOnHost;
    if (at.pending.empty()) return Verdict::kClean;
    const size_t words_at = (size_t)at.st_slots * kStatusBytes;
    std::vector<char> host(words_at + (size_t)at.flags_used * sizeof(int));
    dev.read_bytes(at.st_pool, host.size(), host.data());
    std::vector<StatusRecord> rec((size_t)at.st_used);
    std::vector<int> flags((size_t)at.flags_used);
    if (!rec.empty()) std::memcpy(rec.data(), host.data(), rec.size() * sizeof(StatusRecord));
    if (!flags.empty()) std::memcpy(flags.data(), host.data() + words_at, flags.size() * sizeof(int));
    for (int f : flags)
      if (f & kFlagNonFinite) throw Error(ST_ENUMERIC, "non-finite Gram matrix in orthonormalisation");
    for (const Pending& p : at.pending) {
      for (int i = 0; p.kind == Pending::kOptimisticChol && i < p.npass * p.records_per_pass; ++i)
        if (rec[(size_t)(p.first_record + i)].fail == 3) throw Error(ST_ENUMERIC, "non-finite Gram matrix in orthonormalisation");
      if (p.kind == Pending::kCoreSvd && rec[(size_t)p.record].fail == 3) throw Error(ST_ENUMERIC, "non-finite core matrix in small SVD");
    }
    for (const Pending& p : at.pending) {
      const Verdict v = p.kind == Pending::kRobustChol ? judge_robust_chol(p, flags.data())
                        : p.kind == Pending::kCoreSvd  ? judge_core_svd(p, rec[(size_t)p.record])
                                                       : judge_optimistic_chol(p, &rec[(size_t)p.first_record]);
      if (v != Verdict::kClean) return v;
    }
    return Verdict::kClean;
  }
  Verdict judge_optimistic_chol(const Pending& p, const StatusRecord* r) {
    debug_record(p.first_record, "Cholesky", r[0]);
    const int nrec = p.npass * p.records_per_pass;
    for (int i = 0; i < nrec; ++i)
      if (r[i].fail != 0) return Verdict::kRepeatOnHost;
    for (int i = nrec - p.records_per_pass; p.verify_near_identity && i < nrec; ++i)
      if (!(r[i].dev_i <= 0.25f)) return Verdict::kRepeatOnHost;
    return Verdict::kClean;
  }
  Verdict judge_robust_chol(const Pending& p, const int* flags) {
    if (p.flag_slot < 0) return Verdict::kClean;
    const int* need = flags + p.flag_slot;
    for (int i = p.always; i < p.npass; ++i)
      if (need[i - 1] != 0) ++tm.qr_passes;
    if (std::getenv("CORRLA_DEBUG")) {
      std::fprintf(stderr, "[corrla] device thin-Q: %d passes enqueued, need_next =", p.npass);
      for (int i = 0; i < p.npass; ++i) std::fprintf(stderr, " %d", need[i]);
      const int nrec = p.npass * p.st_per_pass;
      std::vector<int> f2((size_t)nrec);
      std::vector<float> mr((size_t)nrec), di((size_t)nrec);
      dev.read_chol_status(p.st, nrec, f2.data(), mr.data(), di.data());
      std::fprintf(stderr, "; ||G - I||_max / min pivot ratio per factorisation:");
      for (int i = 0; i < nrec; ++i) std::fprintf(stderr, " %.2g/%.2g", di[(size_t)i], mr[(size_t)i]);
      std::fprintf(stderr, "\n");
    }
    return need[p.npass - 1] != 0 ? Verdict::kMorePasses : Verdict::kClean;
  }
  Verdict judge_core_svd(const Pending& p, const StatusRecord& r) {
    debug_record(p.record, "core SVD", r);
    if (r.fail == 0) dev.svd_sweeps_used((int)r.dev_i);
    if (r.fail == 1) return Verdict::kMoreSweeps;
    if (r.fail == 4) return Verdict::kNeedV;
    return r.fail == 0 ? Verdict::kClean : Verdict::kRepeatOnHost;
  }

  void random_svd_tall_body(const TallA<T>& a, int64_t k, int64_t l, int64_t n_iter, const RunOpts& o, Skinny<T>& u_tall,
                            T* s_dev, Skinny<T>& v_tall) {
    PhaseTimer total;
    const bool hh_tmp = qr_householder;
    Skinny<T> q = dev.template alloc_skinny_out<T>(a.mt, l);
    Skinny<T> q2 = hh_tmp ? dev.template alloc_skinny<T>(a.mt, l) : dev.template alloc_skinny_out<T>(a.mt, l);
    power_iter(a, l, n_iter, o, q, q2);
    PhaseTimer pt;
    Skinny<T> bt = dev.template alloc_skinny<T>(a.nt, l);
    mixed_planes_ = o.mixed_project ? o.mixed_planes : 0;
    at_times(a, q, bt, kNone, o.sharded);
    mixed_planes_ = 0;
    phase(tm.project_ms, pt);
    Skinny<T> qb = dev.template alloc_skinny<T>(a.nt, l);
    Skinny<T> qb2 = dev.template alloc_skinny<T>(a.nt, l);
    dev.copy_skinny(bt, qb);
    orthonormalize(qb, qb2, false);
    phase(tm.qr_ms, pt);
    Skinny<T> ct = dev.template alloc_skinny<T>(l, l);
    dev.gemm_nn(as_rowmajor_transposed(bt, l), qb, ct, kNone);
    if (o.poison_core) dev.poison_entry(ct, l / 2, l / 3, o.poison_core);
    Skinny<T> m1 = dev.template alloc_skinny<T>(l, k);
    Skinny<T> m2 = dev.template alloc_skinny<T>(l, k);
    void* svd_st = nullptr;
    if (att_.defer && att_.st_used + 1 <= att_.st_slots) {
      svd_st = status_record(att_.st_used);
      att_.pending.push_back(Pending::core_svd(att_.st_used));
      att_.st_used += 1;
    }
    dev.small_svd(ct, l, k, m2, m1, s_dev, svd_st);
    if (att_.defer) {
      Skinny<T> m1b = dev.template alloc_skinny<T>(l, k);
      orthonormalize_core(m1, m1b, false, true, true);
    }
    if (!att_.defer) {
      std::vector<T> sh((size_t)k);
      dev.copy_values_out(s_dev, k, sh.data(), true);
      const T null_tol = (T)(1e-3 * (double)std::numeric_limits<T>::epsilon()) * sh[0];
      int64_t nz = 0;
      while (nz < k && sh[(size_t)nz] > null_tol) ++nz;
      if (nz < k) complete_basis(m1, nz, false);
      if (nz == k) {
        Skinny<T> m1b = dev.template alloc_skinny<T>(l, k);
        orthonormalize_core(m1, m1b, false, true);
      }
    }
    phase(tm.small_svd_ms, pt);
    dev.gemm_tn(as_rowmajor_transposed(qb, l), m2, v_tall, kNone);
    dev.fix_signs(v_tall, m1, k);
    dev.gemm_tn(as_rowmajor_transposed(q, l), m1, u_tall, kNone);
    phase(tm.finalize_ms, pt);
    tm.host_enqueue_ms += total.lap();
  }

  void phase(double& slot, PhaseTimer& pt) {
    if (profile_phases) dev.sync();
    (void)pt.lap();
    dev.phase_mark(&slot);
  }
  void subphase(double& slot, PhaseTimer& pt) {
    if (!profile_phases) return;
    dev.sync();
    slot += pt.lap();
  }
};

template <class Dev, class T>
inline void small_svd_host(Dev& dev, const Skinny<T>& cd, int64_t l, int64_t k, Skinny<T>& m1, Skinny<T>& m2, T* s_dev) {
  std::vector<double> c((size_t)l * l), uc((size_t)l * l), vc((size_t)l * l), sv(l);
  dev.download_skinny(cd, l, l, c.data());
  const double eps = (double)std::numeric_limits<T>::epsilon();
  if (small::jacobi_svd((int)l, c.data(), (int)l, uc.data(), sv.data(), vc.data(), std::max(1e-15, eps * 1e-3)) < 0)
    throw Error(ST_ENUMERIC, "non-finite core matrix in small SVD");
  dev.upload_skinny(vc.data(), l, k, l, m1);
  dev.upload_skinny(uc.data(), l, k, l, m2);
  std::vector<T> st(k);
  for (int64_t i = 0; i < k; ++i) st[i] = (T)sv[i];
  dev.store_values(st.data(), k, s_dev, false);
}

struct Layout {
  bool fat;
  bool row_major;
  bool needs_pack;
  int64_t mt, nt, ld;
};

inline void validate_matrix(const void* a, int64_t m, int64_t n, int64_t rs, int64_t cs) {
  if (!a) throw Error(ST_EINVAL, "a is NULL");
  if (m < 1 || n < 1) throw Error(ST_EINVAL, "matrix must have at least one row and one column");
  if (rs < 0 || cs < 0) throw Error(ST_EINVAL, "negative strides are not supported");
  if (m > 1 && rs == 0) throw Error(ST_EINVAL, "row_stride == 0 with more than one row");
  if (n > 1 && cs == 0) throw Error(ST_EINVAL, "col_stride == 0 with more than one column");
}

inline Layout classify(int64_t m, int64_t n, int64_t rs, int64_t cs, bool force_tall) {
  Layout L;
  L.fat = !force_tall && m < n;
  L.mt = L.fat ? n : m;
  L.nt = L.fat ? m : n;
// ... 25 lines not shown
```

### corrla_rs_amd/csrc/hip_backend.hpp

```cpp
#pragma once
#include <hip/hip_runtime.h>
#include <rccl/rccl.h>

#include <cmath>
#include <cstdio>
#include <cstdlib>
#include <cstring>
#include <limits>
#include <random>
#include <string>
#include <type_traits>
#include <utility>
#include <vector>

#include "core_svd_plan.hpp"
#include "driver.hpp"
#include "hip_kernels.hpp"
#include "thinq_plan.hpp"
#include "jacobi_mc_kernels.hpp"
#include "ata_kernels.hpp"
#include "tall_kernels.hpp"
#include "mixed_kernels.hpp"
#include "bf16in_kernels.hpp"
#include "grad_kernels.hpp"
// ... 223 lines not shown
  void sync() { CORRLA_HIP(hipStreamSynchronize(stream)); }

  void* alloc_bytes(size_t bytes) {
    bytes = (bytes + 255) / 256 * 256;
    if (bytes == 0) bytes = 256;
    for (auto& c : chunks_)
      if (c.size - c.used >= bytes) {
        void* p = (char*)c.p + c.used;
        c.used += bytes;
        return p;
      }
    Chunk c;
    c.size = std::max<size_t>(bytes, (size_t)64 << 20);
    if (hipMalloc(&c.p, c.size) != hipSuccess) {
      (void)hipGetLastError();
      throw Error(ST_ENOMEM, "device allocation of " + std::to_string(c.size) + " bytes failed");
    }
    c.used = bytes;
    chunks_.push_back(c);
    return c.p;
  }
  void memset_zero(void* p, size_t bytes) { CORRLA_HIP(hipMemsetAsync(p, 0, bytes, stream)); }
  void* alloc_zeroed(size_t bytes) {
    bytes = (bytes + 255) / 256 * 256;
    if (bytes == 0) bytes = 256;
    Chunk* hit = nullptr;
    for (auto& c : zchunks_)
      if (c.size - c.used >= bytes) {
        hit = &c;
        break;
      }
    if (!hit) {
      Chunk c;
      c.size = std::max<size_t>(bytes, (size_t)128 << 20);
      if (hipMalloc(&c.p, c.size) != hipSuccess) {
        (void)hipGetLastError();
        throw Error(ST_ENOMEM, "device allocation of " + std::to_string(c.size) + " bytes failed");
      }
      zchunks_.push_back(c);
      hit = &zchunks_.back();
    }
    char* p = (char*)hit->p + hit->used;
    const size_t end = hit->used + bytes;
    if (end > hit->zeroed) {
      const size_t from = std::max(hit->used, hit->zeroed);
      CORRLA_HIP(hipMemsetAsync((char*)hit->p + from, 0, end - from, stream));
    }
    hit->used = end;
    return p;
  }

  template <class T>
  static Skinny<T> skinny_of(int64_t rows, int64_t cols) {
    const SkinnyLayout lay = skinny_layout(rows, cols);
    Skinny<T> s;
    s.rows = rows;
    s.cols = cols;
    s.ld = lay.ld;
    s.cols_alloc = lay.cols_alloc;
    return s;
  }
  template <class T>
  Skinny<T> alloc_skinny(int64_t rows, int64_t cols) {
    Skinny<T> s = skinny_of<T>(rows, cols);
    const size_t bytes = (size_t)s.ld * (size_t)s.cols_alloc * sizeof(T);
    s.p = (T*)alloc_zeroed(bytes);
    return s;
  }
  template <class T>
  Skinny<T> alloc_skinny_out(int64_t rows, int64_t cols) {
    Skinny<T> s = skinny_of<T>(rows, cols);
    const size_t bytes = (size_t)s.ld * (size_t)s.cols_alloc * sizeof(T);
    if (bytes < ((size_t)4 << 20)) {
      s.p = (T*)alloc_zeroed(bytes);
      return s;
    }
    s.p = (T*)alloc_bytes(bytes);
    if (s.ld > rows)
      CORRLA_HIP(hipMemset2DAsync(s.p + rows, (size_t)s.ld * sizeof(T), 0, (size_t)(s.ld - rows) * sizeof(T), (size_t)s.cols_alloc,
                                  stream));
    if (s.cols_alloc > cols) memset_zero(s.p + cols * s.ld, (size_t)(s.cols_alloc - cols) * s.ld * sizeof(T));
    return s;
  }
  double* alloc_f64(int64_t n) {
    return (double*)alloc_zeroed(sizeof(double) * (size_t)n);
  }
  template <class T>
  T* alloc_scalar(int n) {
    return (T*)alloc_zeroed(sizeof(T) * n);
  }

  void h2d_2d(void* dst, int64_t dpitch_e, const void* src, int64_t spitch_e, int64_t width_e, int64_t rows, size_t esz) {
    CORRLA_HIP(hipMemcpy2DAsync(dst, (size_t)dpitch_e * esz, src, (size_t)spitch_e * esz, (size_t)width_e * esz,
                                (size_t)rows, hipMemcpyHostToDevice, stream));
    sync();
  }
  template <class T>
  void h2d_2d(T* dst, int64_t dpitch_e, const T* src, int64_t spitch_e, int64_t width_e, int64_t rows) {
    h2d_2d((void*)dst, dpitch_e, (const void*)src, spitch_e, width_e, rows, sizeof(T));
  }
  void h2d_2d_enqueue(void* dst, size_t dpitch, const void* src, size_t spitch, size_t width, size_t rows) {
    CORRLA_HIP(hipMemcpy2DAsync(dst, dpitch, src, spitch, width, rows, hipMemcpyHostToDevice, stream));
  }
  void d2d_2d(void* dst, size_t dpitch, const void* src, size_t spitch, size_t width, size_t rows) {
    CORRLA_HIP(hipMemcpy2DAsync(dst, dpitch, src, spitch, width, rows, hipMemcpyDeviceToDevice, stream));
  }
  void d2h_2d(void* dst, size_t dpitch, const void* src, size_t spitch, size_t width, size_t rows) {
    if (rows == 1)
      CORRLA_HIP(hipMemcpyAsync(dst, src, width * rows, hipMemcpyDeviceToHost, stream));
    else
      CORRLA_HIP(hipMemcpy2DAsync(dst, dpitch, src, spitch, width, rows, hipMemcpyDeviceToHost, stream));
  }

  template <class T>
  void gemm_nn(const Big<T>& r, const Skinny<T>& x, Skinny<T>& out, const T* scale_dev);
  template <class T>
  void gemm_tn(const Big<T>& r, const Skinny<T>& x, Skinny<T>& out, const T* scale_dev);

  static constexpr bool kHasSpmm = true;
  template <class T>
  void csr_plan(CsrView<T>& v, bool check_idx);
  template <class T>
  CsrView<T> csr_transpose(const CsrView<T>& a);
  template <class T>
  void spmm(const CsrView<T>& s, const Skinny<T>& x, Skinny<T>& y, const T* scale_dev);
  void* spmm_scratch(size_t bytes) {
    if (bytes > sp_scratch_bytes_) {
      sp_scratch_ = alloc_bytes(bytes);
      sp_scratch_bytes_ = bytes;
    }
    return sp_scratch_;
  }
  void h2d_bytes(void* dst, const void* src, size_t bytes) {
    CORRLA_HIP(hipMemcpyAsync(dst, src, bytes, hipMemcpyHostToDevice, stream));
    sync();
  }

  template <class T>
  bool mixed_fits(bool tn, const Big<T>& r, const Skinny<T>& x, const Skinny<T>& out) const;
  template <class T>
  void gemm_mixed(bool tn, const Big<T>& r, const Skinny<T>& x, Skinny<T>& out, const T* scale_dev, int np);

  static constexpr bool kHasBf16In = true;
  bool bf16a_fits(const Big<uint16_t>& r, int64_t l) const;
  void gemm_bf16a(bool tn, const Big<uint16_t>& r, const Skinny<float>& x, Skinny<float>& out, const float* scale_dev);
  void widen_bf16(const uint16_t* src, int64_t rows, int64_t cols, int64_t rs, int64_t cs, float* dst, int64_t ldd) {
    const int64_t tiles_c = (cols + 31) / 32, tiles_r = (rows + 31) / 32;
    if (tiles_c * tiles_r > 0x7fffffff) throw Error(ST_EINVAL, "problem too large for the launch grid");
    hipLaunchKernelGGL(k::widen_bf16_kernel, dim3((unsigned)(tiles_c * tiles_r)), dim3(256), 0, stream, src, rows, cols, rs, cs, dst, ldd,
                       tiles_c);
    CORRLA_HIP(hipGetLastError());
  }

  template <class T>
  bool ata_fused_fits(const Big<T>& a, int64_t l) const;
  template <class T>
  void ata_fused(const Big<T>& a, const Skinny<T>& x, Skinny<T>& z);

  template <class T>
  void allreduce(T* p, size_t count) {
    if (comm_size <= 1 && !(comm && env_int("CORRLA_FORCE_ALLREDUCE", 0))) return;
    if (!comm) throw Error(ST_ECOMM, "communicator not initialised");
    CORRLA_NCCL(ncclAllReduce(p, p, count, NcclType<T>::v, ncclSum, comm, stream));
    ++n_collectives;
    collective_bytes += (double)count * sizeof(T);
  }
// ... 199 lines not shown
    static_assert(sizeof(k::CholStatus) == 32, "driver.hpp assumes 32-byte status records");
    static_assert(k::kNeedNonFinite == kFlagNonFinite && k::kNeedNullCols == kFlagNullCols, "need_next bits: kernels vs driver");
    std::vector<k::CholStatus> h((size_t)std::max(n, 1));
    CORRLA_HIP(hipMemcpyAsync(h.data(), st_dev, sizeof(k::CholStatus) * n, hipMemcpyDeviceToHost, stream));
    sync();
    for (int i = 0; i < n; ++i) {
      fail[i] = h[i].fail;
      min_ratio[i] = h[i].min_ratio;
      dev_i[i] = h[i].dev_i;
      if (env_int("CORRLA_DEBUG", 0) >= 2)
        std::fprintf(stderr, "[corrla] chol_inv[%d]: fail %d min_ratio %.3g dev_i %.3g clk %lld wall %lld (%.0f MHz)\n", i,
                     h[i].fail, h[i].min_ratio, h[i].dev_i, h[i].clk, h[i].wall,
                     h[i].wall > 0 ? 100.0 * (double)h[i].clk / (double)h[i].wall : 0.0);
    }
  }

  template <class T>
  void inv_sqrt_series(Skinny<T>& g, int64_t r, Skinny<T>& m_out);

  template <class T>
  bool householder_fits(int64_t l) const { return hh_fits(sizeof(T), l); }
  template <class T>
  int householder_max_width() const { return (int)hh_capped_width(hh_max_width(sizeof(T)), thinq_knobs_.hh_block); }
  template <class T>
  struct HhState {
    int64_t m = 0;
    int l = 0;
    HhTreePlan plan;
    std::vector<T*> rbuf, cbuf, taub, vbuf, tbuf;
    T* r_root() const { return rbuf[plan.levels]; }
  };
  template <class T>
  HhState<T> householder_up(Skinny<T>& y, Skinny<T>& tmp);
  template <class T>
  void householder_down(HhState<T>& h, Skinny<T>& y, Skinny<T>& tmp, const T* root_coef = nullptr);
  template <class T>
  void householder_thin_q(Skinny<T>& y, Skinny<T>& tmp) {
    HhState<T> h = householder_up(y, tmp);
    householder_down(h, y, tmp);
  }
  int rank() const { return comm_rank; }

  template <class T>
  void small_svd(const Skinny<T>& c, int64_t l, int64_t k, Skinny<T>& m1, Skinny<T>& m2, T* s_dev, void* conv_status);
  template <class T>
  void copy_out(const Skinny<T>& src, int64_t ncols, T* dst, int64_t ldd, bool transpose, bool to_host) {
    const int64_t rows = src.rows;
    if (!to_host) {
      launch_copy_out(src.p, src.ld, rows, ncols, dst, ldd, transpose);
      return;
    }
    if (!transpose) {
      CORRLA_HIP(hipMemcpy2DAsync(dst, (size_t)ldd * sizeof(T), src.p, (size_t)src.ld * sizeof(T),
                                  (size_t)rows * sizeof(T), (size_t)ncols, hipMemcpyDeviceToHost, stream));
    } else {
      T* tmp = (T*)alloc_bytes((size_t)rows * ncols * sizeof(T));
      launch_copy_out(src.p, src.ld, rows, ncols, tmp, ncols, true);
      CORRLA_HIP(hipMemcpy2DAsync(dst, (size_t)ldd * sizeof(T), tmp, (size_t)ncols * sizeof(T),
                                  (size_t)ncols * sizeof(T), (size_t)rows, hipMemcpyDeviceToHost, stream));
    }
    sync();
  }
  template <class T>
  void pack_strided(const T* src, int64_t rows, int64_t cols, int64_t rs, int64_t cs, T* dst, int64_t ldd) {
    const int64_t tiles_c = (cols + 31) / 32, tiles_r = (rows + 31) / 32;
    if (tiles_c * tiles_r > 0x7fffffff) throw Error(ST_EINVAL, "problem too large for the launch grid");
    dim3 grid((unsigned)(tiles_c * tiles_r));
    hipLaunchKernelGGL((k::pack_strided_kernel<T>), grid, dim3(256), 0, stream, src, rows, cols, rs, cs, dst, ldd, tiles_c);
    CORRLA_HIP(hipGetLastError());
  }

  template <class T>
  void weighted_colsum(const Skinny<T>& x, int64_t rows, const T* w, T* v);
  template <class T>
  void rank1_sub(Skinny<T>& out, int64_t rows, const T* u, const T* v, const T* scale) {
    dim3 grid((unsigned)((rows + 255) / 256), (unsigned)out.cols_alloc);
    check_grid(grid);
    hipLaunchKernelGGL((k::rank1_sub_kernel<T>), grid, dim3(256), 0, stream, out.p, out.ld, rows, u, v, scale);
    CORRLA_HIP(hipGetLastError());
  }

  template <class T>
  void fix_signs(Skinny<T>& v_ref, Skinny<T>& other, int64_t k) {
    hipLaunchKernelGGL((k::column_sign_apply_kernel<T>), dim3((unsigned)k), dim3(256), 0, stream, v_ref.p, v_ref.ld, v_ref.rows,
                       other.p, other.ld, other.rows);
    CORRLA_HIP(hipGetLastError());
  }
  template <class T>
  void fill_const(T* p, int64_t n, T v) {
    const int blocks = (int)std::min<int64_t>(2048, std::max<int64_t>(1, (n + 255) / 256));
    hipLaunchKernelGGL((k::fill_const_kernel<T>), dim3(blocks), dim3(256), 0, stream, p, n, v);
    CORRLA_HIP(hipGetLastError());
  }
  template <class T>
  void center_rows_cols(const T* in, int64_t rows, int64_t cols, int64_t ldi, const T* mu, bool along_cols, T* out,
                        int64_t ldo, const T* inv_sd = nullptr) {
    dim3 grid((unsigned)((cols + 255) / 256), (unsigned)std::min<int64_t>(rows, 4096));
    hipLaunchKernelGGL((k::center_kernel<T>), grid, dim3(256), 0, stream, in, rows, cols, ldi, mu, along_cols ? 1 : 0, out,
                       ldo, inv_sd);
    CORRLA_HIP(hipGetLastError());
  }

  static constexpr bool kHasColVar = true;
  template <class TI, class T>
  void col_ss(const Big<TI>& a, bool along_cols, const T* mu, double* ss);
  template <class T>
  void col_ss_csr(const CsrView<T>& s, const T* mu, int64_t n_samples, double* ss);
  template <class T>
  void sd_from_ss(const double* ss, const T* mu, int64_t n, int64_t m_samples, T* sd, T* inv_sd);
  static constexpr bool kHasSyrk = true;
  const SyrkKnobs& syrk_knobs() const { return syrk_knobs_; }
  static constexpr bool kHasPcaApply = true;
  static constexpr bool kHasRbf = true;
  static constexpr bool kHasPolyfit = true;
  static constexpr bool kHasKde = true;
  static constexpr bool kHasDirichlet = true;
  static constexpr bool kHasMvn = true;
  static constexpr bool kHasLu = true;
  static constexpr bool kHasChol = true;
  const PolyKnobs& poly_knobs() const { return poly_knobs_; }
  const int32_t* poly_table(int64_t kf, int64_t r, int degree) {
    const int64_t key = (kf * 128 + r) * 4 + degree;
    if (key != poly_table_key_) {
      constexpr size_t kMaxBytes = ((size_t)poly_terms(k::kPolyMaxK, 2) + k::kPolyMaxRhs + k::kPolyBT) * sizeof(int32_t);
      if (!poly_table_) CORRLA_HIP(hipMalloc((void**)&poly_table_, kMaxBytes));
      const std::vector<int32_t> t = poly_pair_table(kf, r, degree);
      sync();
      h2d_bytes(poly_table_, t.data(), t.size() * sizeof(int32_t));
      poly_table_key_ = key;
    }
    return poly_table_;
  }
  template <class T>
  void row_scale(const Skinny<T>& in, Skinny<T>& out, int64_t rows, const T* d) {
    if (in.ld != out.ld || in.cols_alloc > out.cols_alloc) throw Error(ST_EINVAL, "internal: row_scale operands must share the padded layout");
    dim3 grid((unsigned)((rows + 255) / 256), (unsigned)in.cols_alloc);
    check_grid(grid);
    hipLaunchKernelGGL((k::row_scale_kernel<T>), grid, dim3(256), 0, stream, (const T*)in.p, out.p, in.ld, rows, d);
    CORRLA_HIP(hipGetLastError());
  }

  template <class T>
  void sumsq(const Skinny<T>& y, double* out_dev) {
    const int64_t n = y.ld * y.cols_alloc;
    const int blocks = (int)std::min<int64_t>(1024, std::max<int64_t>(1, (n + 255) / 256));
    double* partial = (double*)alloc_bytes(sizeof(double) * blocks);
    hipLaunchKernelGGL((k::sumsq_partial_kernel<T>), dim3(blocks), dim3(256), 0, stream, y.p, n, partial);
    hipLaunchKernelGGL(k::sum_partials_kernel, dim3(1), dim3(64), 0, stream, partial, blocks, out_dev);
    CORRLA_HIP(hipGetLastError());
  }
  template <class T>
  void inv_norm(const Skinny<T>& y, double* ss_dev, T* inv_dev) {
    const int64_t n = y.ld * y.cols_alloc;
    const int blocks = (int)std::min<int64_t>(1024, std::max<int64_t>(1, (n + 255) / 256));
    double* partial = (double*)alloc_bytes(sizeof(double) * blocks);
    hipLaunchKernelGGL((k::sumsq_partial_kernel<T>), dim3(blocks), dim3(256), 0, stream, y.p, n, partial);
    hipLaunchKernelGGL((k::sum_partials_rsqrt_kernel<T>), dim3(1), dim3(64), 0, stream, (const double*)partial, blocks, ss_dev, inv_dev);
    CORRLA_HIP(hipGetLastError());
  }
  template <class T>
  void rsqrt_scalar(const double* ss_dev, T* out_dev) {
    hipLaunchKernelGGL((k::rsqrt_scalar_kernel<T>), dim3(1), dim3(1), 0, stream, ss_dev, out_dev);
    CORRLA_HIP(hipGetLastError());
  }
  template <class T>
  void scale_inplace(Skinny<T>& y, const T* scale_dev) {
    const int64_t n = y.ld * y.cols_alloc;
    const int blocks = (int)std::min<int64_t>(2048, std::max<int64_t>(1, (n + 255) / 256));
    hipLaunchKernelGGL((k::scale_kernel<T>), dim3(blocks), dim3(256), 0, stream, y.p, n, scale_dev);
    CORRLA_HIP(hipGetLastError());
  }
  template <class T>
  void fill_normal(T* p, int64_t rows, int64_t cols, int64_t rs, int64_t cs, uint64_t seed, int64_t row0,
                   int64_t global_cols) {
    const int64_t n = rows * cols;
    if (n <= 0) return;
    const int blocks = (int)std::min<int64_t>(8192, (n + 255) / 256);
    hipLaunchKernelGGL((k::fill_normal_kernel<T>), dim3(blocks), dim3(256), 0, stream, p, rows, cols, rs, cs, seed, row0,
                       global_cols, cs <= rs ? 1 : 0);
    CORRLA_HIP(hipGetLastError());
  }

  void set_phase_events(bool on) { phase_events_ = on; }
  void phase_end() {
    if (!phase_events_) phase_mark_impl(nullptr);
  }
  void phase_mark(double* slot) {
    if (!phase_events_ && slot != nullptr) return;
    phase_mark_impl(slot);
  }
  void phase_mark_impl(double* slot) {
    if (ev_used_ == ev_pool_.size()) {
      hipEvent_t e;
      CORRLA_HIP(hipEventCreate(&e));
      ev_pool_.push_back(e);
    }
    hipEvent_t e = ev_pool_[ev_used_++];
    CORRLA_HIP(hipEventRecord(e, stream));
    marks_.push_back({e, slot});
  }
  void phase_forget() {
    for (auto& m_ : marks_) m_.slot = nullptr;
  }
  void phase_resolve(double* total) {
    for (size_t i = 1; i < marks_.size(); ++i) {
      float ms = 0.f;
      if (hipEventElapsedTime(&ms, marks_[i - 1].ev, marks_[i].ev) != hipSuccess) {
        (void)hipGetLastError();
        continue;
      }
      if (marks_[i].slot) *marks_[i].slot += (double)ms;
    }
    if (total && marks_.size() >= 2) {
      float ms = 0.f;
      if (hipEventElapsedTime(&ms, marks_.front().ev, marks_.back().ev) == hipSuccess)
        *total = (double)ms;
      else
        (void)hipGetLastError();
    }
    marks_.clear();
  }

  void event_mark(int i) {
    CORRLA_HIP(hipEventRecord(events_[i], stream));
    events_set_[i] = true;
  }
  double event_elapsed_ms(int i, int j) {
    if (!events_set_[i] || !events_set_[j]) return 0.0;
    float ms = 0.f;
    if (hipEventElapsedTime(&ms, events_[i], events_[j]) != hipSuccess) {
      (void)hipGetLastError();
      return 0.0;
    }
    return (double)ms;
  }

  template <class F>
  double time_on_stream(int reps, F&& f) {
    hipEvent_t e0, e1;
    CORRLA_HIP(hipEventCreate(&e0));
    CORRLA_HIP(hipEventCreate(&e1));
    f();
    CORRLA_HIP(hipEventRecord(e0, stream));
    for (int i = 0; i < reps; ++i) f();
    CORRLA_HIP(hipEventRecord(e1, stream));
    CORRLA_HIP(hipEventSynchronize(e1));
    float ms = 0.f;
    CORRLA_HIP(hipEventElapsedTime(&ms, e0, e1));
    (void)hipEventDestroy(e0);
    (void)hipEventDestroy(e1);
    return (double)ms / reps;
  }

 private:
  struct Chunk {
    void* p = nullptr;
    size_t size = 0, used = 0;
    size_t zeroed = 0;
  };
  std::vector<Chunk> chunks_;
  std::vector<Chunk> zchunks_;
  void* sp_scratch_ = nullptr;
// ... 84 lines not shown
```

### corrla_rs_amd/csrc/hip_kernels.hpp

```cpp
#pragma once
#include <hip/hip_runtime.h>

#include <limits>
#include <stdint.h>

#include <type_traits>

#include "gemm_plan.hpp"
#include "thinq_plan.hpp"

namespace corrla {
namespace k {

typedef float f32x4 __attribute__((ext_vector_type(4)));
typedef double f64x4 __attribute__((ext_vector_type(4)));
typedef double f64x2 __attribute__((ext_vector_type(2)));

#ifndef CORRLA_F32_BIG_IS_A
#define CORRLA_F32_BIG_IS_A true
#endif
template <class T>
struct MT;
template <>
struct MT<float> {
// ... 675 lines not shown
  }
  for (int off = 32; off > 0; off >>= 1) s += __shfl_down(s, off, 64);
  __shared__ double ws[4];
  if ((threadIdx.x & 63) == 0) ws[threadIdx.x >> 6] = s;
  __syncthreads();
  if (threadIdx.x == 0) partial[blockIdx.x] = ws[0] + ws[1] + ws[2] + ws[3];
}
__global__ void sum_partials_kernel(const double* partial, int n, double* out) {
  double s = 0.0;
  for (int i = threadIdx.x; i < n; i += 64) s += partial[i];
  for (int off = 32; off > 0; off >>= 1) s += __shfl_down(s, off, 64);
  if (threadIdx.x == 0) *out = s;
}
template <class T>
__global__ void sum_partials_rsqrt_kernel(const double* partial, int n, double* ss_out, T* inv_out) {
  double s = 0.0;
  for (int i = threadIdx.x; i < n; i += 64) s += partial[i];
  for (int off = 32; off > 0; off >>= 1) s += __shfl_down(s, off, 64);
  if (threadIdx.x == 0) {
    *ss_out = s;
    *inv_out = (T)(s > 0.0 ? 1.0 / sqrt(s) : 0.0);
  }
}
template <class T>
__global__ void rsqrt_scalar_kernel(const double* ss, T* out) {
  const double v = *ss;
  *out = (T)(v > 0.0 ? 1.0 / sqrt(v) : 0.0);
}
template <class T>
__global__ void sub_kernel(T* y, const T* __restrict__ p, int64_t n) {
  for (int64_t i = (int64_t)blockIdx.x * blockDim.x + threadIdx.x; i < n; i += (int64_t)gridDim.x * blockDim.x) y[i] -= p[i];
}
template <class T>
__global__ void scale_kernel(T* y, int64_t n, const T* scale) {
  const T sc = *scale;
  for (int64_t i = (int64_t)blockIdx.x * blockDim.x + threadIdx.x; i < n; i += (int64_t)gridDim.x * blockDim.x)
    y[i] *= sc;
}

__device__ __forceinline__ void philox4x32_10(uint32_t (&c)[4], uint32_t k0, uint32_t k1) {
#pragma unroll
  for (int r = 0; r < 10; ++r) {
    const uint64_t p0 = (uint64_t)0xD2511F53u * c[0];
    const uint64_t p1 = (uint64_t)0xCD9E8D57u * c[2];
    const uint32_t n0 = (uint32_t)(p1 >> 32) ^ c[1] ^ k0;
    const uint32_t n1 = (uint32_t)p1;
    const uint32_t n2 = (uint32_t)(p0 >> 32) ^ c[3] ^ k1;
    const uint32_t n3 = (uint32_t)p0;
    c[0] = n0;
    c[1] = n1;
    c[2] = n2;
    c[3] = n3;
    k0 += 0x9E3779B9u;
    k1 += 0xBB67AE85u;
  }
}
template <class T>
__device__ __forceinline__ T normal_from_index(uint64_t idx, uint64_t seed);
template <>
__device__ __forceinline__ float normal_from_index<float>(uint64_t idx, uint64_t seed) {
  uint32_t c[4] = {(uint32_t)idx, (uint32_t)(idx >> 32), 0u, 0u};
  philox4x32_10(c, (uint32_t)seed, (uint32_t)(seed >> 32));
  const float u1 = ((float)(c[0] >> 8) + 0.5f) * (1.0f / 16777216.0f);
  const float u2 = ((float)(c[1] >> 8) + 0.5f) * (1.0f / 16777216.0f);
  return sqrtf(-2.0f * logf(u1)) * cospif(2.0f * u2);
}
__device__ __forceinline__ void philox_uniform_pair(uint32_t c0, uint32_t c1, uint32_t c2, uint32_t c3, uint64_t seed, double& u1, double& u2) {
  uint32_t c[4] = {c0, c1, c2, c3};
  philox4x32_10(c, (uint32_t)seed, (uint32_t)(seed >> 32));
  const uint64_t a = (((uint64_t)c[0] << 32) | c[1]) >> 11;
  const uint64_t b = (((uint64_t)c[2] << 32) | c[3]) >> 11;
  u1 = ((double)a + 0.5) * (1.0 / 9007199254740992.0);
  u2 = ((double)b + 0.5) * (1.0 / 9007199254740992.0);
}
__device__ __forceinline__ double box_muller_f64(double u1, double u2) { return sqrt(-2.0 * log(u1)) * cospi(2.0 * u2); }
template <>
__device__ __forceinline__ double normal_from_index<double>(uint64_t idx, uint64_t seed) {
  double u1, u2;
  philox_uniform_pair((uint32_t)idx, (uint32_t)(idx >> 32), 0u, 0u, seed, u1, u2);
  return box_muller_f64(u1, u2);
}
template <class T>
__global__ void fill_normal_kernel(T* p, int64_t rows, int64_t cols, int64_t rs, int64_t cs, uint64_t seed, int64_t row0,
                                   int64_t global_cols, int cols_fast) {
  const int64_t total = rows * cols;
  for (int64_t t = (int64_t)blockIdx.x * blockDim.x + threadIdx.x; t < total; t += (int64_t)gridDim.x * blockDim.x) {
    int64_t i, j;
    if (cols_fast) {
      i = t / cols;
      j = t - i * cols;
    } else {
      j = t / rows;
      i = t - j * rows;
    }
    p[i * rs + j * cs] = normal_from_index<T>((uint64_t)((row0 + i) * global_cols + j), seed);
  }
}

template <int G>
__device__ __forceinline__ float group_sum(float x) {
  static_assert(G == 8 || G == 16, "group size");
  auto dpp = [](float v, auto ctrl) {
    return __builtin_bit_cast(float, __builtin_amdgcn_update_dpp(0, __builtin_bit_cast(int, v), decltype(ctrl)::value, 0xf, 0xf, true));
  };
  x += dpp(x, std::integral_constant<int, 0xB1>{});
  x += dpp(x, std::integral_constant<int, 0x4E>{});
  x += dpp(x, std::integral_constant<int, 0x141>{});
  if constexpr (G == 16) x += dpp(x, std::integral_constant<int, 0x140>{});
  return x;
}
template <int G>
__device__ __forceinline__ double group_sum(double x) {
#pragma unroll
  for (int msk = 1; msk < G; msk <<= 1) x += __shfl_xor(x, msk, G);
  return x;
}
template <class T>
__device__ __forceinline__ T jacobi_safe_sigma(T a) {
  return (a >= (T)0 && a < (T)3.0e38) ? (T)sqrt(a) : (T)0;
}
__device__ __forceinline__ bool jacobi_rotation(float a, float b, float g, float tol, float& cs, float& sn, float& rel,
                                                float& t) {
  const float rs = (a > 0.f && b > 0.f) ? __builtin_amdgcn_rsqf(a) * __builtin_amdgcn_rsqf(b) : 0.f;
  rel = fabsf(g) * rs;
  if (!(rel > tol)) return false;
  const float zeta = (b - a) * 0.5f * __builtin_amdgcn_rcpf(g);
  const float den = fabsf(zeta) + __builtin_amdgcn_sqrtf(1.f + zeta * zeta);
  t = copysignf(__builtin_amdgcn_rcpf(den), zeta);
  cs = __builtin_amdgcn_rsqf(1.f + t * t);
  sn = cs * t;
  if (!(fabsf(sn) <= 1.f && cs <= 1.f)) return false;
  return true;
}
__device__ __forceinline__ bool jacobi_rotation(float a, float b, float g, float tol, float& cs, float& sn, float& rel) {
  float t;
  return jacobi_rotation(a, b, g, tol, cs, sn, rel, t);
}
__device__ __forceinline__ double jr_rcp(double x) {
  double y = __builtin_amdgcn_rcp(x);
  return y * (2.0 - x * y);
}
__device__ __forceinline__ double jr_rsq(double x) {
  double y = __builtin_amdgcn_rsq(x);
  return y * (1.5 - 0.5 * x * y * y);
}
__device__ __forceinline__ bool jacobi_rotation(double a, double b, double g, double tol, double& cs, double& sn,
                                                double& rel, double& t) {
  const double rs = (a > 0.0 && b > 0.0) ? jr_rsq(a) * jr_rsq(b) : 0.0;
  rel = fabs(g) * rs;
  if (!(rel > tol)) return false;
  const double zeta = (b - a) * 0.5 * jr_rcp(g);
  const double w = 1.0 + zeta * zeta;
  const double den = fabs(zeta) + w * jr_rsq(w);
  t = copysign(jr_rcp(den), zeta);
  cs = jr_rsq(1.0 + t * t);
  sn = cs * t;
  if (!(fabs(sn) <= 1.0 && cs <= 1.0)) return false;
  return true;
}
__device__ __forceinline__ bool jacobi_rotation(double a, double b, double g, double tol, double& cs, double& sn,
                                                double& rel) {
  double t;
  return jacobi_rotation(a, b, g, tol, cs, sn, rel, t);
}
__device__ __forceinline__ void tournament_pair(int n, int step, int pr, int& p, int& q) {
  if (pr == 0) {
    p = n - 1;
    q = step;
  } else {
    p = step + pr;
    if (p >= n - 1) p -= n - 1;
    q = step - pr;
    if (q < 0) q += n - 1;
  }
  if (p > q) {
    const int t_ = p;
    p = q;
    q = t_;
// ... 579 lines not shown
  for (int off = 32; off > 0; off >>= 1) mx = fmax(mx, __shfl_xor(mx, off, 64));
  if ((threadIdx.x & 63) == 0) red[threadIdx.x >> 6] = mx;
  bad = __syncthreads_or(bad);
  if (threadIdx.x == 0) {
    if (bad) {
      if (st) st->fail = 3;
      if (bad_out) *bad_out = 1;
    }
    if (sexp_out) {
      for (int i = 0; i < 16; ++i) mx = fmax(mx, red[i]);
      int e = 0;
      if (!bad && mx > (T)0 && (mx > (T)1073741824.0 || mx < (T)9.313225746154785e-10)) {
        (void)frexp((double)mx, &e);
        e = 1 - e;
      }
      *sexp_out = e;
    }
  }
}
template <class T>
__global__ void poison_entry_kernel(T* p, int kind) {
  *p = kind == 2 ? std::numeric_limits<T>::infinity() : std::numeric_limits<T>::quiet_NaN();
}

template <class T>
__global__ void fill_const_kernel(T* p, int64_t n, T v) {
  for (int64_t i = (int64_t)blockIdx.x * blockDim.x + threadIdx.x; i < n; i += (int64_t)gridDim.x * blockDim.x) p[i] = v;
}
template <class T>
__global__ void center_kernel(const T* in, int64_t rows, int64_t cols, int64_t ldi, const T* mu, int along_cols, T* out,
                              int64_t ldo, const T* inv_sd) {
  const int64_t c = (int64_t)blockIdx.x * blockDim.x + threadIdx.x;
  if (c >= cols) return;
  const T mc = along_cols ? mu[c] : (T)0;
  const T ic = (inv_sd && along_cols) ? inv_sd[c] : (T)1;
  for (int64_t r = blockIdx.y; r < rows; r += gridDim.y) {
    const T m_ = along_cols ? mc : mu[r];
    const T d = in[r * ldi + c] - m_;
    out[r * ldo + c] = inv_sd ? d * (along_cols ? ic : inv_sd[r]) : d;
  }
}

template <class T>
__global__ __launch_bounds__(256) void wcolsum_partial_kernel(const T* __restrict__ x, int64_t ld, int64_t rows,
                                                              const T* __restrict__ w, double* partial, int ncols) {
  __shared__ double red[256];
  const int c = blockIdx.y;
  const int64_t per = (rows + gridDim.x - 1) / gridDim.x;
  const int64_t r0 = (int64_t)blockIdx.x * per, r1 = min(rows, r0 + per);
  double s = 0.0;
  for (int64_t r = r0 + threadIdx.x; r < r1; r += 256) s += (w ? (double)w[r] : 1.0) * (double)x[(int64_t)c * ld + r];
  red[threadIdx.x] = s;
  __syncthreads();
  for (int off = 128; off > 0; off >>= 1) {
    if ((int)threadIdx.x < off) red[threadIdx.x] += red[threadIdx.x + off];
    __syncthreads();
  }
  if (threadIdx.x == 0) partial[(int64_t)blockIdx.x * ncols + c] = red[0];
}
template <class T>
__global__ void wcolsum_final_kernel(const double* partial, int nblk, int ncols, T* v) {
  const int c = blockIdx.x * blockDim.x + threadIdx.x;
  if (c >= ncols) return;
  double s = 0.0;
  for (int b = 0; b < nblk; ++b) s += partial[(int64_t)b * ncols + c];
  v[c] = (T)s;
}
template <class T>
__global__ void rank1_sub_kernel(T* out, int64_t ld, int64_t rows, const T* __restrict__ u, const T* __restrict__ v,
                                 const T* __restrict__ scale) {
  const int64_t i = (int64_t)blockIdx.x * blockDim.x + threadIdx.x;
  if (i >= rows) return;
  const T sc = scale ? *scale : (T)1;
  out[(int64_t)blockIdx.y * ld + i] -= sc * (u ? u[i] : (T)1) * v[blockIdx.y];
}
template <class T>
__global__ void row_scale_kernel(const T* in, T* out, int64_t ld, int64_t rows, const T* __restrict__ d) {
  const int64_t i = (int64_t)blockIdx.x * blockDim.x + threadIdx.x;
  if (i >= rows) return;
  const int64_t o = (int64_t)blockIdx.y * ld + i;
  out[o] = d[i] * in[o];
}

template <class T>
__global__ __launch_bounds__(256) void column_sign_apply_kernel(T* v, int64_t ld, int64_t rows, T* other, int64_t ld_o, int64_t rows_o) {
  const int j = blockIdx.x;
  T* col = v + (int64_t)j * ld;
  T best = (T)-1;
  int64_t best_i = 0;
  for (int64_t i0 = threadIdx.x; i0 < rows; i0 += 8 * (int64_t)blockDim.x) {
    T a[8];
#pragma unroll
    for (int u = 0; u < 8; ++u) {
      const int64_t i = i0 + u * (int64_t)blockDim.x;
      a[u] = col[i < rows ? i : rows - 1];
    }
#pragma unroll
    for (int u = 0; u < 8; ++u) a[u] = i0 + u * (int64_t)blockDim.x < rows ? (T)fabs(a[u]) : (T)-1;
#pragma unroll
    for (int u = 0; u < 8; ++u)
      if (a[u] > best) {
        best = a[u];
        best_i = i0 + u * (int64_t)blockDim.x;
      }
  }
  __shared__ T sb[256];
  __shared__ int64_t si[256];
  __shared__ int flip;
  sb[threadIdx.x] = best;
  si[threadIdx.x] = best_i;
  __syncthreads();
  for (int off = 128; off > 0; off >>= 1) {
    if ((int)threadIdx.x < off) {
      const T ob = sb[threadIdx.x + off];
      const int64_t oi = si[threadIdx.x + off];
      if (ob > sb[threadIdx.x] || (ob == sb[threadIdx.x] && oi < si[threadIdx.x])) {
        sb[threadIdx.x] = ob;
        si[threadIdx.x] = oi;
      }
    }
    __syncthreads();
  }
  if (threadIdx.x == 0) flip = (sb[0] > (T)0 && col[si[0]] < (T)0) ? 1 : 0;
  __syncthreads();
  if (!flip) return;
  for (int64_t i = threadIdx.x; i < rows; i += blockDim.x) col[i] = -col[i];
  T* oc = other + (int64_t)j * ld_o;
  for (int64_t i = threadIdx.x; i < rows_o; i += blockDim.x) oc[i] = -oc[i];
}

template <class T>
__global__ void pack_strided_kernel(const T* src, int64_t rows, int64_t cols, int64_t rs, int64_t cs, T* dst, int64_t ldd,
                                    int64_t tiles_c) {
  __shared__ T tile[32][33];
  const int64_t r0 = ((int64_t)blockIdx.x / tiles_c) * 32, c0 = ((int64_t)blockIdx.x % tiles_c) * 32;
  const int tx = threadIdx.x & 31, ty = threadIdx.x >> 5;
  const bool col_fast = cs <= rs;
  for (int q = ty; q < 32; q += 8) {
    const int64_t r = col_fast ? r0 + q : r0 + tx;
    const int64_t c = col_fast ? c0 + tx : c0 + q;
    if (r < rows && c < cols) tile[r - r0][c - c0] = src[r * rs + c * cs];
  }
  __syncthreads();
  for (int q = ty; q < 32; q += 8) {
    const int64_t r = r0 + q, c = c0 + tx;
    if (r < rows && c < cols) dst[r * ldd + c] = tile[q][tx];
  }
}
template <class T>
__global__ void copy_out_kernel(const T* src, int64_t lds_, int64_t rows, int64_t cols, T* dst, int64_t ldd, int transpose,
                                int64_t tiles_c) {
  __shared__ T tile[32][33];
  const int64_t r0 = ((int64_t)blockIdx.x / tiles_c) * 32, c0 = ((int64_t)blockIdx.x % tiles_c) * 32;
  const int tx = threadIdx.x & 31, ty = threadIdx.x >> 5;
  if (!transpose) {
    for (int q = ty; q < 32; q += 8) {
      const int64_t r = r0 + tx, c = c0 + q;
      if (r < rows && c < cols) dst[c * ldd + r] = src[c * lds_ + r];
    }
    return;
  }
  for (int q = ty; q < 32; q += 8) {
    const int64_t r = r0 + tx, c = c0 + q;
    if (r < rows && c < cols) tile[q][tx] = src[c * lds_ + r];
  }
  __syncthreads();
  for (int q = ty; q < 32; q += 8) {
    const int64_t r = r0 + q, c = c0 + tx;
    if (r < rows && c < cols) dst[r * ldd + c] = tile[tx][q];
  }
}

}
}
```

### include/corrla_rsvd.h

```cpp
#ifndef CORRLA_RSVD_H
#define CORRLA_RSVD_H

#include <stddef.h>
#include <stdint.h>

#ifdef __cplusplus
extern "C" {
#endif

#if defined(__GNUC__)
#define CORRLA_API __attribute__((visibility("default")))
#else
#define CORRLA_API
#endif

typedef struct corrla_ctx corrla_ctx;

typedef enum corrla_status {
  CORRLA_OK = 0,
  CORRLA_EINVAL = 1,
  CORRLA_ENOMEM = 2,
  CORRLA_EHIP = 3,
  CORRLA_ECOMM = 4,
  CORRLA_ENUMERIC = 5,
// ... 270 lines not shown
CORRLA_API corrla_status corrla_poly_eval_f64(corrla_ctx* ctx, const double* x, int64_t m, int64_t k, int64_t ldx, const double* coeffs,
                                              int64_t ldc, int64_t r, int degree, double* out, int64_t ld_out, double* jac, int64_t ld_jac);
CORRLA_API corrla_status corrla_poly_eval_dev_f32(corrla_ctx* ctx, const float* x, int64_t m, int64_t k, int64_t ldx, const double* coeffs,
                                                  int64_t ldc, int64_t r, int degree, float* out, int64_t ld_out, float* jac, int64_t ld_jac);
CORRLA_API corrla_status corrla_poly_eval_dev_f64(corrla_ctx* ctx, const double* x, int64_t m, int64_t k, int64_t ldx, const double* coeffs,
                                                  int64_t ldc, int64_t r, int degree, double* out, int64_t ld_out, double* jac, int64_t ld_jac);
CORRLA_API corrla_status corrla_ctx_last_polyfit(corrla_ctx* ctx, int* route_out);

CORRLA_API corrla_status corrla_kde_eval_f32(corrla_ctx* ctx, const float* x, int64_t n_q, int64_t incx, const float* s, int64_t n_s,
                                             int64_t incs, double h, int what, float* out, int64_t inco);
CORRLA_API corrla_status corrla_kde_eval_f64(corrla_ctx* ctx, const double* x, int64_t n_q, int64_t incx, const double* s, int64_t n_s,
                                             int64_t incs, double h, int what, double* out, int64_t inco);
CORRLA_API corrla_status corrla_kde_eval_dev_f32(corrla_ctx* ctx, const float* x, int64_t n_q, int64_t incx, const float* s, int64_t n_s,
                                                 int64_t incs, double h, int what, float* out, int64_t inco);
CORRLA_API corrla_status corrla_kde_eval_dev_f64(corrla_ctx* ctx, const double* x, int64_t n_q, int64_t incx, const double* s, int64_t n_s,
                                                 int64_t incs, double h, int what, double* out, int64_t inco);
CORRLA_API corrla_status corrla_kde_nll_f32(corrla_ctx* ctx, const float* x, int64_t n_t, int64_t incx, const float* s, int64_t n_s,
                                            int64_t incs, const double* h, int64_t n_h, double* nll, double* dnll);
CORRLA_API corrla_status corrla_kde_nll_f64(corrla_ctx* ctx, const double* x, int64_t n_t, int64_t incx, const double* s, int64_t n_s,
                                            int64_t incs, const double* h, int64_t n_h, double* nll, double* dnll);
CORRLA_API corrla_status corrla_kde_nll_dev_f32(corrla_ctx* ctx, const float* x, int64_t n_t, int64_t incx, const float* s, int64_t n_s,
                                                int64_t incs, const double* h, int64_t n_h, double* nll, double* dnll);
CORRLA_API corrla_status corrla_kde_nll_dev_f64(corrla_ctx* ctx, const double* x, int64_t n_t, int64_t incx, const double* s, int64_t n_s,
                                                int64_t incs, const double* h, int64_t n_h, double* nll, double* dnll);
CORRLA_API corrla_status corrla_ctx_last_kde(corrla_ctx* ctx, int* route_out);

CORRLA_API corrla_status corrla_lu_solve_f64(corrla_ctx* ctx, const double* a, int64_t n, int64_t lda, const double* b, int64_t n_rhs,
                                             int64_t ldb, double* x, int64_t ldx);
CORRLA_API corrla_status corrla_lu_solve_dev_f64(corrla_ctx* ctx, double* a, int64_t n, int64_t lda, double* b, int64_t n_rhs, int64_t ldb,
                                                 int64_t* ipiv);
CORRLA_API corrla_status corrla_rbffit_system_f64(corrla_ctx* ctx, const double* xs, int64_t n_s, int64_t ldxs, int64_t dim, int kernel,
                                               double eps, int poly_degree, double* m, int64_t ldm);
CORRLA_API corrla_status corrla_rbffit_system_dev_f64(corrla_ctx* ctx, const double* xs, int64_t n_s, int64_t ldxs, int64_t dim, int kernel,
                                                   double eps, int poly_degree, double* m, int64_t ldm);
CORRLA_API corrla_status corrla_rbffit_f64(corrla_ctx* ctx, const double* xs, int64_t n_s, int64_t ldxs, int64_t dim, const double* y,
                                            int64_t n_rhs, int64_t ldy, int kernel, double eps, int poly_degree, double* coeffs, int64_t ldw);
CORRLA_API corrla_status corrla_rbffit_dev_f64(corrla_ctx* ctx, const double* xs, int64_t n_s, int64_t ldxs, int64_t dim, const double* y,
                                                int64_t n_rhs, int64_t ldy, int kernel, double eps, int poly_degree, double* coeffs,
                                                int64_t ldw);
CORRLA_API corrla_status corrla_ctx_last_solve(corrla_ctx* ctx, int* route, int64_t* info, double* min_pivot, double* max_u);

CORRLA_API corrla_status corrla_chol_factor_f64(corrla_ctx* ctx, const double* a, int64_t n, int64_t lda, double* l, int64_t ldl);
CORRLA_API corrla_status corrla_chol_factor_dev_f64(corrla_ctx* ctx, double* a, int64_t n, int64_t lda);
CORRLA_API corrla_status corrla_chol_solve_f64(corrla_ctx* ctx, const double* a, int64_t n, int64_t lda, const double* b, int64_t n_rhs,
                                               int64_t ldb, double* x, int64_t ldx);
CORRLA_API corrla_status corrla_chol_solve_dev_f64(corrla_ctx* ctx, double* a, int64_t n, int64_t lda, double* b, int64_t n_rhs, int64_t ldb);
CORRLA_API corrla_status corrla_ctx_last_chol(corrla_ctx* ctx, int* route, int64_t* info, double* min_diag, double* max_diag, double* logdet);

CORRLA_API corrla_status corrla_dirichlet_draws_f64(corrla_ctx* ctx, const double* alphas, int64_t d, double c_scale, uint64_t seed,
                                                    int64_t first, int64_t n, double* out, int64_t ldo);
CORRLA_API corrla_status corrla_dirichlet_draws_dev_f64(corrla_ctx* ctx, const double* alphas, int64_t d, double c_scale, uint64_t seed,
                                                        int64_t first, int64_t n, double* out, int64_t ldo);
CORRLA_API corrla_status corrla_dirichlet_sample_f64(corrla_ctx* ctx, const double* bounds, const double* alphas, int64_t d, double c_scale,
                                                     uint64_t seed, int64_t n_samples, int64_t max_zshots, int64_t chunk_size, double* out,
                                                     int64_t ldo, int64_t* n_found, int64_t* n_drawn);
CORRLA_API corrla_status corrla_dirichlet_sample_dev_f64(corrla_ctx* ctx, const double* bounds, const double* alphas, int64_t d, double c_scale,
                                                         uint64_t seed, int64_t n_samples, int64_t max_zshots, int64_t chunk_size, double* out,
                                                         int64_t ldo, int64_t* n_found, int64_t* n_drawn);
CORRLA_API corrla_status corrla_ctx_last_dirichlet(corrla_ctx* ctx, int* route_out);

CORRLA_API corrla_status corrla_mvn_sample_f32(corrla_ctx* ctx, int64_t n, int64_t d, int64_t r, const float* factor, int64_t ldf,
                                               const float* mean, uint64_t seed, int64_t first, int lower, float* out, int64_t ldo);
CORRLA_API corrla_status corrla_mvn_sample_f64(corrla_ctx* ctx, int64_t n, int64_t d, int64_t r, const double* factor, int64_t ldf,
                                               const double* mean, uint64_t seed, int64_t first, int lower, double* out, int64_t ldo);
CORRLA_API corrla_status corrla_mvn_sample_dev_f32(corrla_ctx* ctx, int64_t n, int64_t d, int64_t r, const float* factor, int64_t ldf,
                                                   const float* mean, uint64_t seed, int64_t first, int lower, float* out, int64_t ldo);
CORRLA_API corrla_status corrla_mvn_sample_dev_f64(corrla_ctx* ctx, int64_t n, int64_t d, int64_t r, const double* factor, int64_t ldf,
                                                   const double* mean, uint64_t seed, int64_t first, int lower, double* out, int64_t ldo);
CORRLA_API corrla_status corrla_sandwich_diag_f32(corrla_ctx* ctx, const float* jac, int64_t m, int64_t d, int64_t ldj, const float* cov,
                                                  int64_t ldc, float* v);
CORRLA_API corrla_status corrla_sandwich_diag_f64(corrla_ctx* ctx, const double* jac, int64_t m, int64_t d, int64_t ldj, const double* cov,
                                                  int64_t ldc, double* v);
CORRLA_API corrla_status corrla_sandwich_diag_dev_f32(corrla_ctx* ctx, const float* jac, int64_t m, int64_t d, int64_t ldj, const float* cov,
                                                      int64_t ldc, float* v);
CORRLA_API corrla_status corrla_sandwich_diag_dev_f64(corrla_ctx* ctx, const double* jac, int64_t m, int64_t d, int64_t ldj, const double* cov,
                                                      int64_t ldc, double* v);
CORRLA_API corrla_status corrla_ctx_last_mvn(corrla_ctx* ctx, int* route_out);

CORRLA_API corrla_status corrla_fill_normal_dev_f32(corrla_ctx* ctx, float* p, int64_t rows, int64_t cols, int64_t row_stride,
                                         int64_t col_stride, uint64_t seed, int64_t row0, int64_t global_cols);
CORRLA_API corrla_status corrla_fill_normal_dev_f64(corrla_ctx* ctx, double* p, int64_t rows, int64_t cols, int64_t row_stride,
                                         int64_t col_stride, uint64_t seed, int64_t row0, int64_t global_cols);

CORRLA_API corrla_status corrla_grad_mat_f64(corrla_ctx* ctx, const double* x, int64_t n_pts, int64_t k, const double* y,
                                             const double* xq, int64_t n_q, int est_order, int64_t n_nbrs, double out_scale,
                                             double* g, int64_t ldg, int* n_regularised);
CORRLA_API corrla_status corrla_grad_mat_dev_f64(corrla_ctx* ctx, const double* x, int64_t n_pts, int64_t k, const double* y,
                                                 const double* xq, int64_t n_q, int est_order, int64_t n_nbrs,
                                                 double out_scale, double* g, int64_t ldg, int* n_regularised);

CORRLA_API corrla_status corrla_time_sketch_dev_f32(corrla_ctx* ctx, const float* a, int64_t m, int64_t n, int64_t row_stride,
                                         int64_t col_stride, const float* x, int64_t ldx, int64_t l, float* y,
                                         int64_t ldy, int reps, double* avg_ms);
CORRLA_API corrla_status corrla_time_sketch_dev_f64(corrla_ctx* ctx, const double* a, int64_t m, int64_t n, int64_t row_stride,
                                         int64_t col_stride, const double* x, int64_t ldx, int64_t l, double* y,
                                         int64_t ldy, int reps, double* avg_ms);

#define CORRLA_UNIQUE_ID_BYTES 128
CORRLA_API corrla_status corrla_comm_unique_id(void* out128);
CORRLA_API corrla_status corrla_ctx_comm_init(corrla_ctx* ctx, const void* unique_id128, int rank, int nranks);

CORRLA_API corrla_status corrla_rsvd_sharded_dev_f32(corrla_ctx* ctx, const float* a_local, int64_t m_local, int64_t n,
                                          int64_t row_stride, int64_t col_stride, int64_t rank, int64_t n_iter,
                                          int64_t n_oversamples, const corrla_opts* opts, float* u_local, int64_t ldu,
                                          float* s, float* vt, int64_t ldvt);
CORRLA_API corrla_status corrla_rsvd_sharded_dev_f64(corrla_ctx* ctx, const double* a_local, int64_t m_local, int64_t n,
                                          int64_t row_stride, int64_t col_stride, int64_t rank, int64_t n_iter,
                                          int64_t n_oversamples, const corrla_opts* opts, double* u_local, int64_t ldu,
                                          double* s, double* vt, int64_t ldvt);

#ifdef __cplusplus
}
#endif
#endif
```

Measured before the change: 95070.

## Trim allocation zeroing, copies and memsets across RSVD driver and sign fix

Output skinny buffers that exactly fill whole column tiles are now allocated without a zeroing memset, and the omega fill writes zeros into its padding columns itself. Singular values go straight into the caller's buffer, so a separate copy-out is skipped. The B-transpose copy before orthonormalisation is replaced by having the first CholQR pass read from the source directly. The conv-status memset is skipped for the multi-workgroup SVD path. The column sign kernel switches to wave shuffles with a larger block and unrolled flips. A new fix_signs C API is added. These cut memsets, copies and launches, but they rely on every consumer fully overwriting buffers that are no longer zeroed.

Measured after the change: 94880. No clear change (-0.2%).

```diff
diff --git a/corrla_rs_amd/_lib.py b/corrla_rs_amd/_lib.py
--- a/corrla_rs_amd/_lib.py
+++ b/corrla_rs_amd/_lib.py
@@ -133,6 +133,7 @@
         s["corrla_mvn_sample_" + suf] = s["corrla_mvn_sample_dev_" + suf] = (C.c_int, [vp, i64, i64, i64, vp, i64, vp, u64, i64, C.c_int, vp, i64])
         s["corrla_sandwich_diag_" + suf] = s["corrla_sandwich_diag_dev_" + suf] = (C.c_int, [vp, vp, i64, i64, i64, vp, i64, vp])
         s["corrla_fill_normal_dev_" + suf] =(C.c_int, [vp, vp, i64, i64, i64, i64, u64, i64, i64])
+        s["corrla_fix_signs_dev_" + suf] = (C.c_int, [vp, vp, i64, i64, i64, vp, i64, i64])
         s["corrla_time_sketch_dev_" + suf] = (C.c_int, [vp, vp, i64, i64, i64, i64, vp, i64, i64, vp, i64, C.c_int,
                                                          C.POINTER(dbl)])
     s["corrla_rsvd_bf16"] = s["corrla_rsvd_dev_bf16"] = s["corrla_rsvd_f32"]
diff --git a/corrla_rs_amd/api.py b/corrla_rs_amd/api.py
--- a/corrla_rs_amd/api.py
+++ b/corrla_rs_amd/api.py
@@ -1106,6 +1106,14 @@
                    int(global_cols if global_cols is not None else cols)))
         return t
 
+    def fix_signs(self, v, other):
+        k, n = v.shape
+        assert v.is_contiguous() and other.is_contiguous() and other.shape[0] == k and other.dtype == v.dtype
+        _sync_stream(v)
+        fn = self._entry("corrla_fix_signs_", True, v.dtype)
+        L.check(fn(self._h, v.data_ptr(), n, n, k, other.data_ptr(), other.shape[1], other.shape[1]))
+        return v, other
+
     def time_sketch(self, a, x, reps=10):
         import torch
         m, n = a.shape
diff --git a/corrla_rs_amd/csrc/capi_impl.hpp b/corrla_rs_amd/csrc/capi_impl.hpp
--- a/corrla_rs_amd/csrc/capi_impl.hpp
+++ b/corrla_rs_amd/csrc/capi_impl.hpp
@@ -246,9 +246,9 @@
         l = std::min<int64_t>(c.rank + c.n_oversamples, ta.nt);
         if (ro.omega && ro.omega_ld < ta.nt) throw Error(ST_EINVAL, "omega_ld < min(m, n)");
         u_in_place = !c.fat && !c.host_ptrs && !c.empty_shard;
-        ut = u_in_place ? caller_skinny(c.u, ta.mt, k, c.ldu) : dev.template alloc_skinny<T>(ta.mt, k);
-        vtall = dev.template alloc_skinny<T>(ta.nt, k);
-        s_dev = dev.template alloc_scalar<T>((int)k);
+        ut = u_in_place ? caller_skinny(c.u, ta.mt, k, c.ldu) : alloc_product_out<T>(dev, ta.mt, k, true, false);
+        vtall = alloc_product_out<T>(dev, ta.nt, k, true, false);
+        s_dev = c.host_ptrs ? dev.template alloc_scalar<T>((int)k) : c.s;
       });
   RsvdDriver<Dev, T> drv(dev, c.profile);
   if (c.empty_shard) drv.m_local_override_ = 0;
@@ -260,7 +260,7 @@
       dev.copy_out(vtall, k, c.u, c.ldu, false, c.host_ptrs);
       if (!c.empty_shard) dev.copy_out(ut, k, c.vt, c.ldvt, true, c.host_ptrs);
     }
-    dev.copy_values_out(s_dev, k, c.s, c.host_ptrs);
+    if (s_dev != c.s) dev.copy_values_out(s_dev, k, c.s, c.host_ptrs);
   });
   finish_call(drv, dev, c.tm_out, true);
 }
diff --git a/corrla_rs_amd/csrc/core_svd_stage.hpp b/corrla_rs_amd/csrc/core_svd_stage.hpp
--- a/corrla_rs_amd/csrc/core_svd_stage.hpp
+++ b/corrla_rs_amd/csrc/core_svd_stage.hpp
@@ -184,9 +184,9 @@
 
 template <class T>
 void HipDev::small_svd(const Skinny<T>& c, int64_t l, int64_t k, Skinny<T>& m1, Skinny<T>& m2, T* s_dev, void* conv_status) {
-  if (conv_status) memset_zero(conv_status, sizeof(k::CholStatus));
   const CoreSvdCall<T> a{c, l, k, m1, m2, s_dev, conv_status};
   const CoreSvdPlan plan = core_svd_plan((int)sizeof(T), l, k, core_svd_stage::knobs_from_env(), svd_state_, conv_status != nullptr);
+  if (conv_status && plan.family != CoreSvd::kMultiWg) memset_zero(conv_status, sizeof(k::CholStatus));
   switch (plan.family) {
     case CoreSvd::kMultiWg:
       core_svd_stage::multi_wg(*this, a, plan);
diff --git a/corrla_rs_amd/csrc/corrla_rsvd.hip b/corrla_rs_amd/csrc/corrla_rsvd.hip
--- a/corrla_rs_amd/csrc/corrla_rsvd.hip
+++ b/corrla_rs_amd/csrc/corrla_rsvd.hip
@@ -79,6 +79,22 @@
     std::lock_guard<std::mutex> lk(c->mu);
     CORRLA_HIP(hipSetDevice(c->dev.device));
     c->dev.fill_normal(p, rows, cols, rs, cs, seed, row0, global_cols);
+    c->dev.sync();
+  });
+}
+template <class T>
+corrla_status fix_signs_c(corrla_ctx* ctx, T* v, int64_t ldv, int64_t n, int64_t k, T* other, int64_t ld_other, int64_t rows_other) {
+  return guarded([&] {
+    corrla_ctx* c = need(ctx);
+    if (!v || !other) throw Error(ST_EINVAL, "v or other is NULL");
+    if (n < 1 || k < 1 || rows_other < 1 || ldv < n || ld_other < rows_other) throw Error(ST_EINVAL, "bad fix_signs shape");
+    if (k > 0x7fffffff) throw Error(ST_EINVAL, "fix_signs: too many columns for the launch grid");
+    std::lock_guard<std::mutex> lk(c->mu);
+    CORRLA_HIP(hipSetDevice(c->dev.device));
+    Skinny<T> vs, os;
+    vs.p = v, vs.rows = n, vs.cols = vs.cols_alloc = k, vs.ld = ldv, vs.external = true;
+    os.p = other, os.rows = rows_other, os.cols = os.cols_alloc = k, os.ld = ld_other, os.external = true;
+    c->dev.fix_signs(vs, os, k);
     c->dev.sync();
   });
 }
@@ -214,6 +230,10 @@
                                              int64_t cs, uint64_t seed, int64_t row0, int64_t global_cols) {           \
     return fill_c<T>(ctx, p, rows, cols, rs, cs, seed, row0, global_cols);                                             \
   }                                                                                                                    \
+  CORRLA_API corrla_status corrla_fix_signs_dev_##SUF(corrla_ctx* ctx, T* v, int64_t ldv, int64_t n, int64_t k, T* other,          \
+                                             int64_t ld_other, int64_t rows_other) {                                   \
+    return fix_signs_c<T>(ctx, v, ldv, n, k, other, ld_other, rows_other);                                             \
+  }                                                                                                                    \
   CORRLA_API corrla_status corrla_time_sketch_dev_##SUF(corrla_ctx* ctx, const T* a, int64_t m, int64_t n, int64_t rs,            \
                                              int64_t cs, const T* x, int64_t ldx, int64_t l, T* y, int64_t ldy,        \
                                              int reps, double* avg_ms) {                                               \
diff --git a/corrla_rs_amd/csrc/driver.hpp b/corrla_rs_amd/csrc/driver.hpp
--- a/corrla_rs_amd/csrc/driver.hpp
+++ b/corrla_rs_amd/csrc/driver.hpp
@@ -121,6 +121,25 @@
 struct dev_has_chol : std::false_type {};
 template <class D>
 struct dev_has_chol<D, std::void_t<decltype(D::kHasChol)>> : std::true_type {};
+
+template <class D, class = void>
+struct dev_has_whole_tile_out : std::false_type {};
+template <class D>
+struct dev_has_whole_tile_out<D, std::void_t<decltype(D::kHasWholeTileOut)>> : std::true_type {};
+
+template <class T, class Dev>
+inline Skinny<T> alloc_product_out(Dev& dev, int64_t rows, int64_t cols, bool whole_tiles, bool out_before) {
+  if constexpr (dev_has_whole_tile_out<Dev>::value)
+    if (whole_tiles && Dev::whole_tile_fill(rows, cols)) return dev.template alloc_skinny_whole<T>(rows, cols);
+  return out_before ? dev.template alloc_skinny_out<T>(rows, cols) : dev.template alloc_skinny<T>(rows, cols);
+}
+template <class T, class Dev>
+inline void fill_omega(Dev& dev, Skinny<T>& om, uint64_t seed) {
+  if constexpr (dev_has_whole_tile_out<Dev>::value)
+    dev.fill_normal(om.p, om.rows, om.cols, (int64_t)1, om.ld, seed, (int64_t)0, om.cols, om.cols_alloc - om.cols);
+  else
+    dev.fill_normal(om.p, om.rows, om.cols, (int64_t)1, om.ld, seed, (int64_t)0, om.cols);
+}
 
 template <class T>
 struct TallA {
@@ -383,16 +402,17 @@
     }
   }
 
-  int64_t orthonormalize(Skinny<T>& y, Skinny<T>& tmp, bool sharded, bool rough = false) {
+  int64_t orthonormalize(Skinny<T>& y, Skinny<T>& tmp, bool sharded, bool rough = false, const Skinny<T>* src = nullptr) {
     const int64_t l = y.cols;
     if (householder_usable(y, sharded)) {
+      if (src) dev.copy_skinny(*src, y);
       PhaseTimer qt0;
       householder_thin_q_any_width(y, tmp, sharded);
       ++tm.qr_passes;
       subphase(tm.qr_gram_ms, qt0);
       return l;
     }
-    int64_t r = orthonormalize_core(y, tmp, sharded, rough);
+    int64_t r = orthonormalize_core(y, tmp, sharded, rough, false, src);
     if (r < l && !att_.defer && (sharded ? global_rows(true) : y.rows) >= l) r = complete_basis(y, r, sharded);
     return r;
   }
@@ -418,13 +438,17 @@
   }
 
   template <class Factor>
-  void cholqr_pass(Skinny<T>& y, Skinny<T>& tmp, Skinny<T>& gd, bool sharded, bool inplace, Factor&& factor) {
+  void cholqr_pass(Skinny<T>& y, Skinny<T>& tmp, Skinny<T>& gd, bool sharded, bool inplace, Factor&& factor,
+                   const Skinny<T>* src = nullptr) {
     const int64_t l = y.cols;
-    Skinny<T> yv = y.view_cols(l);
-    dev.gemm_nn(as_rowmajor_transposed(y, l), yv, gd, kNone);
+    const Skinny<T>& in = src ? *src : y;
+    Skinny<T> yv = in.view_cols(l);
+    dev.gemm_nn(as_rowmajor_transposed(in, l), yv, gd, kNone);
     if (sharded) dev.allreduce(gd.p, (size_t)gd.ld * (size_t)gd.cols_alloc);
     const Skinny<T> md = factor(gd);
-    if (inplace) {
+    if (inplace && src) {
+      dev.gemm_tn(as_rowmajor_transposed(in, l), md, y, kNone);
+    } else if (inplace) {
       dev.apply_inplace(y, l, md);
     } else {
       dev.gemm_tn(as_rowmajor_transposed(y, l), md, tmp, kNone);
@@ -470,10 +494,15 @@
     dev.copy_block(x22, 0, 0, n2, n2, md, n1, n1);
   }
 
-  int64_t orthonormalize_device(Skinny<T>& y, Skinny<T>& tmp, bool sharded, bool rough, bool polish) {
+  int64_t orthonormalize_device(Skinny<T>& y, Skinny<T>& tmp, bool sharded, bool rough, bool polish,
+                                const Skinny<T>* src = nullptr) {
     const int64_t l = y.cols;
     PhaseTimer qt0;
     const bool inplace = dev.qr_inplace_fits(l), single = dev.template device_chol_fits<T>(l);
+    if (src && !inplace) {
+      dev.copy_skinny(*src, y);
+      src = nullptr;
+    }
     const RobustSchedule sched =
         robust_schedule(dev.robust_passes(), polish ? RobustMode::kPolish : (rough ? RobustMode::kInLoop : RobustMode::kFinal), inplace);
     const int npass = sched.npass, always = sched.always;
@@ -507,7 +536,7 @@
         });
         dev.template combine_need<T>(need + pass, ps.need_ratio > 0.f ? nullptr : insp, need_blk, need_blk + 1);
         return md;
-      });
+      }, pass == 0 ? src : nullptr);
       if (ps.refill)
         dev.refill_null(y, l, null_mask, (uint64_t)(0x9e3779b97f4a7c15ull ^ (uint64_t)(977 * (att_.flags_used + pass) + l)));
       if (pass < always) ++tm.qr_passes;
@@ -520,12 +549,14 @@
     return l;
   }
 
-  int64_t orthonormalize_core(Skinny<T>& y, Skinny<T>& tmp, bool sharded, bool rough, bool polish = false) {
+  int64_t orthonormalize_core(Skinny<T>& y, Skinny<T>& tmp, bool sharded, bool rough, bool polish = false,
+                              const Skinny<T>* src = nullptr) {
     const int64_t l = y.cols;
     int64_t r = l;
     if (att_.defer && (sharded || y.rows >= l) && att_.flags_used + kRobustPasses <= att_.flags_cap &&
         dev.template device_qr_robust_fits<T>(l))
-      return orthonormalize_device(y, tmp, sharded, rough, polish);
+      return orthonormalize_device(y, tmp, sharded, rough, polish, src);
+    if (src) dev.copy_skinny(*src, y);
     const int rpp = records_per_pass(l);
     if (rpp > 0) {
       PhaseTimer qt0;
@@ -678,16 +709,16 @@
       ~MixedScope() { slot = saved; }
     } mixed_scope(mixed_planes_, o.mixed_planes);
     PhaseTimer pt;
-    Skinny<T> om = dev.template alloc_skinny<T>(a.nt, l);
+    Skinny<T> om = !o.omega ? alloc_product_out<T>(dev, a.nt, l, true, false) : dev.template alloc_skinny<T>(a.nt, l);
     if (o.omega) {
       if (o.omega_on_device)
         dev.copy_in_skinny((const T*)o.omega, o.omega_ld, om);
       else
         dev.upload_skinny_native((const T*)o.omega, o.omega_ld, om);
     } else {
-      dev.fill_normal(om.p, a.nt, l, 1, om.ld, o.seed, 0, l);
-    }
-    Skinny<T> z = dev.template alloc_skinny<T>(a.nt, l);
+      fill_omega(dev, om, o.seed);
+    }
+    Skinny<T> z = alloc_product_out<T>(dev, a.nt, l, !a.sparse, false);
     double* ss_dev = dev.alloc_f64(1);
     T* inv_dev = dev.template alloc_scalar<T>(1);
     int64_t i0 = 0;
@@ -857,19 +888,18 @@
                             T* s_dev, Skinny<T>& v_tall) {
     PhaseTimer total;
     const bool hh_tmp = qr_householder;
-    Skinny<T> q = dev.template alloc_skinny_out<T>(a.mt, l);
-    Skinny<T> q2 = hh_tmp ? dev.template alloc_skinny<T>(a.mt, l) : dev.template alloc_skinny_out<T>(a.mt, l);
+    Skinny<T> q = alloc_product_out<T>(dev, a.mt, l, !a.sparse, true);
+    Skinny<T> q2 = hh_tmp ? dev.template alloc_skinny<T>(a.mt, l) : alloc_product_out<T>(dev, a.mt, l, true, true);
     power_iter(a, l, n_iter, o, q, q2);
     PhaseTimer pt;
-    Skinny<T> bt = dev.template alloc_skinny<T>(a.nt, l);
+    Skinny<T> bt = alloc_product_out<T>(dev, a.nt, l, !a.sparse, false);
     mixed_planes_ = o.mixed_project ? o.mixed_planes : 0;
     at_times(a, q, bt, kNone, o.sharded);
     mixed_planes_ = 0;
     phase(tm.project_ms, pt);
-    Skinny<T> qb = dev.template alloc_skinny<T>(a.nt, l);
-    Skinny<T> qb2 = dev.template alloc_skinny<T>(a.nt, l);
-    dev.copy_skinny(bt, qb);
-    orthonormalize(qb, qb2, false);
+    Skinny<T> qb = alloc_product_out<T>(dev, a.nt, l, true, false);
+    Skinny<T> qb2 = hh_tmp ? dev.template alloc_skinny<T>(a.nt, l) : alloc_product_out<T>(dev, a.nt, l, true, false);
+    orthonormalize(qb, qb2, false, false, &bt);
     phase(tm.qr_ms, pt);
     Skinny<T> ct = dev.template alloc_skinny<T>(l, l);
     dev.gemm_nn(as_rowmajor_transposed(bt, l), qb, ct, kNone);
diff --git a/corrla_rs_amd/csrc/hip_backend.hpp b/corrla_rs_amd/csrc/hip_backend.hpp
--- a/corrla_rs_amd/csrc/hip_backend.hpp
+++ b/corrla_rs_amd/csrc/hip_backend.hpp
@@ -329,6 +329,18 @@
     if (s.cols_alloc > cols) memset_zero(s.p + cols * s.ld, (size_t)(s.cols_alloc - cols) * s.ld * sizeof(T));
     return s;
   }
+  static constexpr bool kHasWholeTileOut = true;
+  static bool whole_tile_fill(int64_t rows, int64_t cols) {
+    const SkinnyLayout lay = skinny_layout(rows, cols);
+    return lay.ld == rows && lay.cols_alloc == (int64_t)col_blocking(cols).tiles * 16;
+  }
+  template <class T>
+  Skinny<T> alloc_skinny_whole(int64_t rows, int64_t cols) {
+    Skinny<T> s = skinny_of<T>(rows, cols);
+    const size_t bytes = (size_t)s.ld * (size_t)s.cols_alloc * sizeof(T);
+    s.p = (T*)(bytes < ((size_t)4 << 20) ? alloc_zeroed(bytes) : alloc_bytes(bytes));
+    return s;
+  }
   double* alloc_f64(int64_t n) {
     return (double*)alloc_zeroed(sizeof(double) * (size_t)n);
   }
@@ -694,7 +706,8 @@
 
   template <class T>
   void fix_signs(Skinny<T>& v_ref, Skinny<T>& other, int64_t k) {
-    hipLaunchKernelGGL((k::column_sign_apply_kernel<T>), dim3((unsigned)k), dim3(256), 0, stream, v_ref.p, v_ref.ld, v_ref.rows,
+    const int threads = (int)std::min<int64_t>(k::kSignThreads, std::max<int64_t>(256, round_up((v_ref.rows + 7) / 8, 64)));
+    hipLaunchKernelGGL((k::column_sign_apply_kernel<T>), dim3((unsigned)k), dim3(threads), 0, stream, v_ref.p, v_ref.ld, v_ref.rows,
                        other.p, other.ld, other.rows);
     CORRLA_HIP(hipGetLastError());
   }
@@ -784,12 +797,12 @@
   }
   template <class T>
   void fill_normal(T* p, int64_t rows, int64_t cols, int64_t rs, int64_t cs, uint64_t seed, int64_t row0,
-                   int64_t global_cols) {
-    const int64_t n = rows * cols;
+                   int64_t global_cols, int64_t zero_cols = 0) {
+    const int64_t n = rows * (cols + zero_cols);
     if (n <= 0) return;
     const int blocks = (int)std::min<int64_t>(8192, (n + 255) / 256);
     hipLaunchKernelGGL((k::fill_normal_kernel<T>), dim3(blocks), dim3(256), 0, stream, p, rows, cols, rs, cs, seed, row0,
-                       global_cols, cs <= rs ? 1 : 0);
+                       global_cols, cs <= rs ? 1 : 0, zero_cols);
     CORRLA_HIP(hipGetLastError());
   }
 
diff --git a/corrla_rs_amd/csrc/hip_kernels.hpp b/corrla_rs_amd/csrc/hip_kernels.hpp
--- a/corrla_rs_amd/csrc/hip_kernels.hpp
+++ b/corrla_rs_amd/csrc/hip_kernels.hpp
@@ -781,18 +781,18 @@
 }
 template <class T>
 __global__ void fill_normal_kernel(T* p, int64_t rows, int64_t cols, int64_t rs, int64_t cs, uint64_t seed, int64_t row0,
-                                   int64_t global_cols, int cols_fast) {
-  const int64_t total = rows * cols;
+                                   int64_t global_cols, int cols_fast, int64_t zero_cols = 0) {
+  const int64_t ctot = cols + zero_cols, total = rows * ctot;
   for (int64_t t = (int64_t)blockIdx.x * blockDim.x + threadIdx.x; t < total; t += (int64_t)gridDim.x * blockDim.x) {
     int64_t i, j;
     if (cols_fast) {
-      i = t / cols;
-      j = t - i * cols;
+      i = t / ctot;
+      j = t - i * ctot;
     } else {
       j = t / rows;
       i = t - j * rows;
     }
-    p[i * rs + j * cs] = normal_from_index<T>((uint64_t)((row0 + i) * global_cols + j), seed);
+    p[i * rs + j * cs] = j < cols ? normal_from_index<T>((uint64_t)((row0 + i) * global_cols + j), seed) : (T)0;
   }
 }
 
@@ -1538,8 +1538,10 @@
   out[o] = d[i] * in[o];
 }
 
-template <class T>
-__global__ __launch_bounds__(256) void column_sign_apply_kernel(T* v, int64_t ld, int64_t rows, T* other, int64_t ld_o, int64_t rows_o) {
+constexpr int kSignThreads = 1024;
+template <class T>
+__global__ __launch_bounds__(kSignThreads) void column_sign_apply_kernel(T* v, int64_t ld, int64_t rows, T* other, int64_t ld_o,
+                                                                         int64_t rows_o) {
   const int j = blockIdx.x;
   T* col = v + (int64_t)j * ld;
   T best = (T)-1;
@@ -1560,27 +1562,46 @@
         best_i = i0 + u * (int64_t)blockDim.x;
       }
   }
-  __shared__ T sb[256];
-  __shared__ int64_t si[256];
+  auto take = [&](T ob, int64_t oi) {
+    if (ob > best || (ob == best && oi < best_i)) {
+      best = ob;
+      best_i = oi;
+    }
+  };
+  for (int off = 32; off > 0; off >>= 1) {
+    const T ob = __shfl_down(best, off, 64);
+    const long long oi = __shfl_down((long long)best_i, off, 64);
+    take(ob, (int64_t)oi);
+  }
+  constexpr int kWaves = kSignThreads / 64;
+  __shared__ T sb[kWaves];
+  __shared__ int64_t si[kWaves];
   __shared__ int flip;
-  sb[threadIdx.x] = best;
-  si[threadIdx.x] = best_i;
+  const int wave = threadIdx.x >> 6, nwaves = (int)(blockDim.x >> 6);
+  if ((threadIdx.x & 63) == 0) {
+    sb[wave] = best;
+    si[wave] = best_i;
+  }
   __syncthreads();
-  for (int off = 128; off > 0; off >>= 1) {
-    if ((int)threadIdx.x < off) {
-      const T ob = sb[threadIdx.x + off];
-      const int64_t oi = si[threadIdx.x + off];
-      if (ob > sb[threadIdx.x] || (ob == sb[threadIdx.x] && oi < si[threadIdx.x])) {
-        sb[threadIdx.x] = ob;
-        si[threadIdx.x] = oi;
-      }
-    }
-    __syncthreads();
-  }
-  if (threadIdx.x == 0) flip = (sb[0] > (T)0 && col[si[0]] < (T)0) ? 1 : 0;
+  if (threadIdx.x == 0) {
+    for (int w = 1; w < nwaves; ++w) take(sb[w], si[w]);
+    flip = (best > (T)0 && col[best_i] < (T)0) ? 1 : 0;
+  }
   __syncthreads();
   if (!flip) return;
-  for (int64_t i = threadIdx.x; i < rows; i += blockDim.x) col[i] = -col[i];
+  for (int64_t i0 = threadIdx.x; i0 < rows; i0 += 8 * (int64_t)blockDim.x) {
+    T a[8];
+#pragma unroll
+    for (int u = 0; u < 8; ++u) {
+      const int64_t i = i0 + u * (int64_t)blockDim.x;
+      a[u] = col[i < rows ? i : rows - 1];
+    }
+#pragma unroll
+    for (int u = 0; u < 8; ++u) {
+      const int64_t i = i0 + u * (int64_t)blockDim.x;
+      if (i < rows) col[i] = -a[u];
+    }
+  }
   T* oc = other + (int64_t)j * ld_o;
   for (int64_t i = threadIdx.x; i < rows_o; i += blockDim.x) oc[i] = -oc[i];
 }
diff --git a/include/corrla_rsvd.h b/include/corrla_rsvd.h
--- a/include/corrla_rsvd.h
+++ b/include/corrla_rsvd.h
@@ -376,6 +376,11 @@
 CORRLA_API corrla_status corrla_fill_normal_dev_f64(corrla_ctx* ctx, double* p, int64_t rows, int64_t cols, int64_t row_stride,
                                          int64_t col_stride, uint64_t seed, int64_t row0, int64_t global_cols);
 
+CORRLA_API corrla_status corrla_fix_signs_dev_f32(corrla_ctx* ctx, float* v, int64_t ldv, int64_t n, int64_t k, float* other,
+                                       int64_t ld_other, int64_t rows_other);
+CORRLA_API corrla_status corrla_fix_signs_dev_f64(corrla_ctx* ctx, double* v, int64_t ldv, int64_t n, int64_t k, double* other,
+                                       int64_t ld_other, int64_t rows_other);
+
 CORRLA_API corrla_status corrla_grad_mat_f64(corrla_ctx* ctx, const double* x, int64_t n_pts, int64_t k, const double* y,
                                              const double* xq, int64_t n_q, int est_order, int64_t n_nbrs, double out_scale,
                                              double* g, int64_t ldg, int* n_regularised);
```
